# NVlabs/gbrl

Hardware: AMD Instinct MI355X
Metric: trees-fit/sec + predict rows/sec at batch=2^20, feat=128, depth=6, out=8 (higher is better)
Workload: dtype int32 fixed-point sums / f32 scores

## Files before the change

### gbrl_amd/csrc/engine_candidates.hip

```cpp
#include "engine_step_detail.h"

namespace gbrl {

namespace detail {

void spin_until_published(volatile uint32_t *flag, uint32_t seq, hipStream_t s, const char *what) {
    const double kSpinSeconds = [] { const char *e = hooks::raw(hooks::SPIN_SECONDS); const double v = e ? std::atof(e) : 0.0; return v > 0.0 ? v : 120.0; }();
    int idle = 0;
    std::chrono::steady_clock::time_point t0;
    bool timed = false;
    for (unsigned spins = 1; *flag != seq; ++spins) {
        if ((spins & 0x3fff) == 0) {
            const hipError_t q = hipStreamQuery(s);
            if (q == hipSuccess) { if (++idle > 64) throw HipError(std::string("internal: ") + what + " were not published"); }
            else if (q != hipErrorNotReady) hip_check(q, what);
            if (!timed) { t0 = std::chrono::steady_clock::now(); timed = true; }
            else if (std::chrono::duration<double>(std::chrono::steady_clock::now() - t0).count() > kSpinSeconds) {
                hip_check(hipStreamSynchronize(s), what);
                if (*flag == seq) break;
                throw HipError(std::string("timeout: ") + what + " did not arrive (stream drained, nothing published)");
            }
        }
    }
    std::atomic_thread_fence(std::memory_order_acquire);
// ... 412 lines not shown
        kern::fetch_segments(fs, s);
        cat_table_.valid = true; cat_table_.keys = d_keys; cat_table_.slot_q = d_slotq; cat_table_.cls_of_q = dc; cat_table_.log2_cap = log2_cap;
        if (cat_prof) {
            cp[4] = std::chrono::steady_clock::now();
            auto us = [](std::chrono::steady_clock::time_point a, std::chrono::steady_clock::time_point b) { return std::chrono::duration<double, std::micro>(b - a).count(); };
            fprintf(stderr, "[cat host, us] %d distinct: insertion order %.1f  items %.1f  container order %.1f  candidates + classes %.1f\n", n_distinct, us(cp[0], cp[1]), us(cp[1], cp[2]), us(cp[2], cp[3]), us(cp[3], cp[4]));
        }
        return true;
    }
    struct DictE { uint64_t h; int cls; int item; };
    std::vector<DictE> ent(n_ent);
    std::vector<int32_t> off(Fc + 1, 0);
    for (int q : cand_item) ++off[lfeat[q] + 1];
    for (int f = 0; f < Fc; ++f) off[f + 1] += off[f];
    {
        std::vector<int32_t> cur(off.begin(), off.end() - 1);
        cat_cands.reserve(cat_cands.size() + n_ent);
        for (int q : cand_item) {
            const int f = lfeat[q];
            const int cls = ++cat_classes[f];
            if (cls > 65534) throw Unsupported("more than 65534 candidate categories in one feature");
            cat_cands.emplace_back(f, cat_items_[item_of_q[q]].name, cls);
            ent[cur[f]++] = {lhash[q], cls, q};
        }
    }
    for (int f = 0; f < Fc; ++f)
        std::sort(ent.begin() + off[f], ent.begin() + off[f + 1], [](const DictE &a, const DictE &b2) { return a.h < b2.h || (a.h == b2.h && a.cls < b2.cls); });
    const size_t n1 = static_cast<size_t>(n_ent) + 1;
    const size_t o_words = 0, o_hash = o_words + n1 * kCat, o_off = o_hash + n1 * 8, o_cls = o_off + (static_cast<size_t>(Fc) + 1) * 4,
                 dict_bytes = o_cls + n1 * 4;
    char *hd = static_cast<char *>(pin_cat_dict_.ensure((dict_bytes + 3) & ~static_cast<size_t>(3)));
    for (int e = 0; e < n_ent; ++e) {
        std::memcpy(hd + o_words + static_cast<size_t>(e) * kCat, names + static_cast<size_t>(ent[e].item) * kCat, kCat);
        reinterpret_cast<uint64_t *>(hd + o_hash)[e] = ent[e].h;
        reinterpret_cast<int32_t *>(hd + o_cls)[e] = ent[e].cls;
    }
    std::memset(hd + o_words + static_cast<size_t>(n_ent) * kCat, 0, kCat);
    reinterpret_cast<uint64_t *>(hd + o_hash)[n_ent] = 0;
    reinterpret_cast<int32_t *>(hd + o_cls)[n_ent] = 0;
    std::memcpy(hd + o_off, off.data(), (static_cast<size_t>(Fc) + 1) * 4);
    char *dd = static_cast<char *>(d_sdict_.ensure((dict_bytes + 3) & ~static_cast<size_t>(3)));
    {
        void *hd_dev = nullptr;
        hip_check(hipHostGetDevicePointer(&hd_dev, hd, 0), "hipHostGetDevicePointer");
        kern::FetchSegments fs{};
        fs.n = 1; fs.dst[0] = dd; fs.src[0] = hd_dev; fs.words[0] = static_cast<uint32_t>((dict_bytes + 3) / 4);
        kern::fetch_segments(fs, s);
    }
    sdict_words_ = reinterpret_cast<const uint64_t *>(dd + o_words);
    sdict_hash_ = reinterpret_cast<const uint64_t *>(dd + o_hash);
    sdict_off_ = reinterpret_cast<const int32_t *>(dd + o_off);
    sdict_cls_ = reinterpret_cast<const int32_t *>(dd + o_cls);
    return true;
}

void Engine::verify_pending_categories() {
    bool clash = false;
    for (const auto &pq : cat_pending_) clash = clash || std::memcmp(cat_items_[pq.first].name, pq.second, kCat) != 0;
    if (!cat_pending_.empty() && hooks::on(hooks::TEST_CAT_CLASH)) clash = true;
    cat_pending_.clear();
    if (clash) cat_clash_ = true;
}

int64_t *Engine::quantile_cum_device(const std::vector<int64_t> &cum, long long n_global, int B) {
    hipStream_t s = stream_;
    const bool grown = d_cum_.capacity() < sizeof(int64_t) * static_cast<size_t>(B);
    int64_t *d_cum = static_cast<int64_t *>(d_cum_.ensure(sizeof(int64_t) * B));
    if (grown || cum_cache_n_ != n_global || cum_cache_b_ != B) {
        int64_t *h = static_cast<int64_t *>(pin_cum_.ensure(sizeof(int64_t) * B));
        std::memcpy(h, cum.data(), sizeof(int64_t) * B);
        hip_check(hipMemcpyAsync(d_cum, h, sizeof(int64_t) * B, hipMemcpyHostToDevice, s), "H2D cum");
        hip_check(hipStreamSynchronize(s), "sync cum");
        cum_cache_n_ = n_global;
        cum_cache_b_ = B;
    }
    return d_cum;
}
void Engine::numeric_thresholds(const float *dobs, int N, int F, int B, long long n_global, const uint32_t *d_kt, float *d_thr,
                                uint32_t *d_thrkeys, int pass1_chunks, uint16_t *d_codes_out, bool *codes_written) {
    if (codes_written) *codes_written = false;
    hipStream_t s = stream_;
    const gbrl_hip_metadata &md = model.meta;
    uint32_t *d_qflags = static_cast<uint32_t *>(d_qflags_.ensure(sizeof(uint32_t) * 4));
    bool fast_quantile = false;
    auto upload_cum = [&](const std::vector<int64_t> &cum) -> int64_t * { return quantile_cum_device(cum, n_global, B); };
    auto bisection_quantiles = [&](const std::vector<int64_t> &cum) {
        int64_t *d_cum = upload_cum(cum);
        uint32_t *d_prefix = static_cast<uint32_t *>(d_prefix_.ensure(sizeof(uint32_t) * F * B));
        uint32_t *d_trial = static_cast<uint32_t *>(d_trial_.ensure(sizeof(uint32_t) * F * B));
        int64_t *d_counts = static_cast<int64_t *>(d_counts_.ensure(sizeof(int64_t) * F * (B + 1)));
        kern::qsel_init(d_prefix, d_trial, F, B, s);
        for (int bit = 31; bit >= 0; --bit) {
            hip_check(hipMemsetAsync(d_counts, 0, sizeof(int64_t) * F * (B + 1), s), "memset");
            kern::bin_rows(dobs, N, F, d_trial, B, false, d_counts, nullptr, 0, 0, s);
            if (has_coll_) exchange(Red::SumI64, d_counts, static_cast<size_t>(F) * (B + 1));
            kern::qsel_update(d_prefix, d_trial, d_counts, d_cum, F, B, bit, bit - 1, s);
        }
        hip_check(hipMemcpyAsync(d_thrkeys, d_trial, sizeof(uint32_t) * F * B, hipMemcpyDeviceToDevice, s), "D2D keys");
    };
    std::vector<int64_t> cum;
    if (F > 0 && !fixed_thr_.empty()) {
        if (fixed_thr_.size() != static_cast<size_t>(F) * B) throw HipError("internal: fixed thresholds do not match this model");
        hip_check(hipMemcpyAsync(d_thr, fixed_thr_.data(), sizeof(float) * fixed_thr_.size(), hipMemcpyHostToDevice, s), "H2D thresholds");
        kern::floats_to_keys(d_thr, d_thrkeys, fixed_thr_.size(), s);
    } else if (F > 0) {
        if (md.generator_type == GBRL_HIP_GEN_UNIFORM) {
            uint32_t *d_mm = static_cast<uint32_t *>(d_minmax_.ensure(sizeof(uint32_t) * 2 * F));
            {
                kern::FillSegments fz{};
                fz.n = 2;
                fz.dst[0] = d_mm; fz.words[0] = static_cast<uint32_t>(F); fz.value[0] = 0xffffffffu;
                fz.dst[1] = d_mm + F; fz.words[1] = static_cast<uint32_t>(F); fz.value[1] = 0u;
                kern::fill_segments(fz, s);
            }
            kern::column_minmax(d_kt, N, F, d_mm, d_mm + F, s);
            if (has_coll_) {
                float *tmp = static_cast<float *>(d_trial_.ensure(sizeof(float) * 2 * F));
                kern::keys_to_floats(d_mm, tmp, 2 * static_cast<size_t>(F), s);
                kern::negate_f32(tmp, F, s);
                exchange(Red::MaxF32, tmp, 2 * static_cast<size_t>(F));
                kern::negate_f32(tmp, F, s);
                kern::floats_to_keys(tmp, d_mm, 2 * static_cast<size_t>(F), s);
            }
            kern::uniform_thresholds(d_mm, d_mm + F, F, B, d_thr, s, d_thrkeys);
        } else {
            cum = quantile_target_ranks(n_global, B);
            bool floats_done = false;
            const bool coll_fast = has_coll_ && (coll_.world_size & (coll_.world_size - 1)) == 0 && coll_.world_size <= 8;
            const bool radix_ok = !force_sample_select_ && B <= kern::radix_max_targets() && n_global < (1ll << 32);
            if (force_bisection_ || (has_coll_ && !coll_fast && !radix_ok)) {
                bisection_quantiles(cum);
            } else if (!has_coll_ && !force_sample_select_ && !force_radix_ && kern::sort_quantiles_fits(N, B)) {
                int64_t *d_cum = upload_cum(cum);
                const bool no_fuse = [] { const char *e = hooks::raw(hooks::SORT_NO_CODES); return e && e[0] == '1'; }();
                uint16_t *cdst = no_fuse ? nullptr : d_codes_out;
                kern::sort_quantiles(d_kt, N, F, d_cum, B, d_thrkeys, d_thr, s, cdst);
                if (cdst && codes_written) *codes_written = true;
                floats_done = true;
                last_quantile_fallback_ = false;
            } else if (!force_sample_select_ && B <= kern::radix_max_targets() && n_global < (1ll << 32)) {
                int64_t *d_cum = upload_cum(cum);
                void *d_rs = d_radix_state_.ensure(kern::radix_state_bytes(F, B));
                uint32_t *d_rp = static_cast<uint32_t *>(d_radix_partial_.ensure(kern::radix_partial_bytes(F)));
                uint32_t *d_rl = static_cast<uint32_t *>(d_qlists_.ensure(kern::radix_list_bytes(N, F)));
                kern::RadixComm comm{};
                if (has_coll_) {
                    comm.ctx = this;
                    comm.allreduce_sum_i64 = &Engine::radix_exchange_trampoline;
                    comm.stream_ordered = rccl_comm_ != nullptr;
                    comm.gbuf = static_cast<int64_t *>(d_counts_.ensure(sizeof(int64_t) * kern::radix_exchange_words(F)));
                    comm.partial_global = static_cast<uint32_t *>(d_radix_global_.ensure(kern::radix_global_partial_bytes(F)));
                }
                uint32_t *d_le = has_coll_ ? nullptr : static_cast<uint32_t *>(d_root_le_.ensure(sizeof(uint32_t) * (static_cast<size_t>(F) * B + F)));
                const int rc = kern::radix_select(d_kt, N, F, d_cum, B, d_rs, d_rp, d_rl, d_thrkeys, s, has_coll_ ? &comm : nullptr, pass1_chunks, d_le);
                root_le_ = d_le;
                if (rc != 0) throw HipError(rc == 2 ? "allreduce failed" : "radix select failed");
                last_quantile_fallback_ = false;
            } else {
                fast_quantile = true;
                kern::QuantilePlan plan = kern::quantile_plan(N);
                if (has_coll_) { plan.sample = 4096; plan.n_split = kern::kQuantileMaxSplit; }
                const size_t all_keys = static_cast<size_t>(N) * F;
                const uint32_t max_elems = static_cast<uint32_t>(B > 256 ? all_keys : std::min<size_t>(all_keys, std::max<size_t>(1u << 20, all_keys / 4)));
                int64_t *d_cum = upload_cum(cum);
                uint32_t *d_split = static_cast<uint32_t *>(d_splitters_.ensure(sizeof(uint32_t) * 2 * static_cast<size_t>(F) * kern::kQuantileMaxSplit));
                uint32_t *d_split_bfs = d_split + static_cast<size_t>(F) * kern::kQuantileMaxSplit;
                uint32_t *d_cc = static_cast<uint32_t *>(d_ccounts_.ensure(sizeof(uint32_t) * static_cast<size_t>(plan.n_chunks) * F * kern::kQuantileClasses));
                uint32_t *d_coff = static_cast<uint32_t *>(d_c2l_.ensure(sizeof(uint32_t) * F * kern::kQuantileClasses));
                uint32_t *d_toff = static_cast<uint32_t *>(d_tgt_list_.ensure(sizeof(uint32_t) * 2 * static_cast<size_t>(F) * B));
                uint32_t *d_tlen = d_toff + static_cast<size_t>(F) * B;
                uint32_t *d_tr = static_cast<uint32_t *>(d_tgt_rank_.ensure(sizeof(uint32_t) * F * B));
                uint32_t *d_lists = static_cast<uint32_t *>(d_qlists_.ensure(sizeof(uint32_t) * max_elems));
                hip_check(hipMemsetAsync(d_coff, 0xff, sizeof(uint32_t) * F * kern::kQuantileClasses, s), "memset");
                hip_check(hipMemsetAsync(d_qflags, 0, sizeof(uint32_t) * 4, s), "memset");
                int64_t *d_gcounts = nullptr;
                if (has_coll_) {
                    const int S = 4096, SU = S * coll_.world_size;
                    uint32_t *d_samp = static_cast<uint32_t *>(d_prefix_.ensure(sizeof(uint32_t) * static_cast<size_t>(F) * S));
                    int64_t *d_uni = static_cast<int64_t *>(d_counts_.ensure(sizeof(int64_t) * std::max<size_t>(static_cast<size_t>(F) * SU, static_cast<size_t>(F) * kern::kQuantileClasses)));
                    kern::sample_only(d_kt, N, F, S, d_samp, s);
                    hip_check(hipMemsetAsync(d_uni, 0, sizeof(int64_t) * static_cast<size_t>(F) * SU, s), "memset");
                    kern::place_sample(d_samp, F, S, coll_.rank, SU, d_uni, s);
                    exchange(Red::SumI64, d_uni, static_cast<size_t>(F) * SU);
                    kern::union_splitters(d_uni, F, SU, plan.n_split, d_split, d_split_bfs, s);
                    kern::class_count(d_kt, N, F, plan, d_split_bfs, d_cc, s);
                    d_gcounts = d_uni;
                    kern::counts_to_i64(d_cc, plan.n_chunks, static_cast<size_t>(F) * kern::kQuantileClasses, d_gcounts, s);
                    exchange(Red::SumI64, d_gcounts, static_cast<size_t>(F) * kern::kQuantileClasses);
                } else {
                    kern::sample_splitters(d_kt, N, F, plan, d_split, d_split_bfs, s);
                    hip_check(hipGetLastError(), "sample_splitters launch");
                    kern::class_count(d_kt, N, F, plan, d_split_bfs, d_cc, s);
                    hip_check(hipGetLastError(), "class_count launch");
                }
                kern::quantile_targets(d_cc, d_gcounts, d_split, d_cum, F, B, plan, d_coff, d_toff, d_tlen, d_tr, d_thrkeys, d_qflags, max_elems,
                                       d_qflags + 2, s);
                kern::quantile_extract(d_kt, N, F, plan, d_split_bfs, d_coff, d_cc, d_lists, s);
                hip_check(hipGetLastError(), "quantile_extract launch");
                if (has_coll_) {
                    uint32_t *d_pref = static_cast<uint32_t *>(d_trial_.ensure(sizeof(uint32_t) * static_cast<size_t>(F) * B));
                    int64_t *d_scnt = static_cast<int64_t *>(d_selcnt_.ensure(sizeof(int64_t) * (static_cast<size_t>(F) * B + 1)));
                    hip_check(hipMemsetAsync(d_pref, 0, sizeof(uint32_t) * static_cast<size_t>(F) * B, s), "memset");
                    for (int bit = 31; bit >= 0; --bit) {
                        kern::select_count(d_lists, d_toff, d_tlen, d_pref, bit, F * B, d_scnt, s);
                        hip_check(hipGetLastError(), "select_count launch");
                        exchange(Red::SumI64, d_scnt, static_cast<size_t>(F) * B);
                        kern::select_update(d_pref, d_scnt, d_toff, d_tr, bit, F * B, d_thrkeys, s);
                        hip_check(hipGetLastError(), "select_update launch");
                    }
                } else {
                    kern::quantile_select(d_lists, d_toff, d_tlen, d_tr, F * B, d_thrkeys, s);
                    hip_check(hipGetLastError(), "quantile_select launch");
                }
            }
            if (!floats_done) kern::keys_to_floats(d_thrkeys, d_thr, static_cast<size_t>(F) * B, s);
        }
        uint32_t qflags[4] = {0, 0, 0, 0};
        if (fast_quantile) {
            hip_check(hipMemcpyAsync(qflags, d_qflags, sizeof(qflags), hipMemcpyDeviceToHost, s), "D2H flags");
            hip_check(hipStreamSynchronize(s), "sync");
            if (has_coll_) {
                int64_t *d_flag = static_cast<int64_t *>(d_selcnt_.ensure(sizeof(int64_t) * 2));
                int64_t hv = qflags[2];
                hip_check(hipMemcpyAsync(d_flag, &hv, sizeof(hv), hipMemcpyHostToDevice, s), "H2D flag");
                exchange(Red::SumI64, d_flag, 1);
                hip_check(hipMemcpyAsync(&hv, d_flag, sizeof(hv), hipMemcpyDeviceToHost, s), "D2H flag");
                hip_check(hipStreamSynchronize(s), "sync");
                qflags[2] = hv != 0;
            }
            if (qflags[2] != 0) {
                bisection_quantiles(cum);
                kern::keys_to_floats(d_thrkeys, d_thr, static_cast<size_t>(F) * B, s);
                last_quantile_fallback_ = true;
            } else {
                last_quantile_fallback_ = false;
            }
        }
    }
}

}
```

### gbrl_amd/csrc/engine_grow_levels.hip

```cpp
#include "engine_grow_detail.h"

namespace gbrl {

using namespace detail;

void Engine::grow_levels(const GrowCtx &c, const GrowDims &dims, const StepTables &t, TreeBuilder &tb, std::vector<int64_t> &acc, double &leaf_scale) {
    hipStream_t s = stream_;
    const bool device_plan = c.oblivious && !has_coll_ && device_levels_requested() && c.MD > 0 && c.MD <= 11  &&
                             c.n_cand > 0 && !dims.l2_degenerate;
    Stager sta(pin_a_, d_stage_a_, dims.stage_bytes, s), stb(pin_b_, d_stage_b_, dims.stage_bytes, s);
    LevelWork w = level_workspace(c, dims);
    tb.reset(dims.max_nodes);
    kern::publish_pair(c.d_thr, c.pub_thr_dev, c.pub_thr_bytes, c.d_scales, c.pub_scales_dev, sizeof(kern::StepScales), s);
    if (device_plan) grow_levels_planned(c, dims, t, w, tb);
    else if (c.n_cand > 0 && !dims.l2_degenerate) grow_levels_host(c, dims, t, w, tb, sta, stb);
    finish_leaves(c, dims, w, tb, sta, acc, leaf_scale);
}

LevelWork Engine::level_workspace(const GrowCtx &c, const GrowDims &dims) {
    hipStream_t s = stream_;
    const int N = c.N, D = c.D, max_front = dims.max_front;
    LevelWork w{};
    w.rows[0] = static_cast<int32_t *>(d_rows_[0].ensure(sizeof(int32_t) * N));
    w.rows[1] = static_cast<int32_t *>(d_rows_[1].ensure(sizeof(int32_t) * N));
// ... 173 lines not shown
    L.active = std::move(active);
    const std::vector<int> &act = L.active;
    const int n_act = L.n_act = static_cast<int>(act.size());
    L.d_hist = w.hist_lvl[depth & 1];
    L.d_hist_prev = w.hist_lvl[(depth & 1) ^ 1];
    std::vector<int> &compute_ids = L.compute_ids;
    std::vector<int32_t> &slot_map = L.slot_map, sub_par(n_act, -1), sub_sib(n_act, -1);
    if (depth == 0) {
        compute_ids = act;
        for (int k = 0; k < n_act; ++k) slot_map.push_back(k);
    } else {
        std::vector<int> slot_of(nodes.size(), -1);
        for (int k = 0; k < n_act; ++k) slot_of[act[k]] = k;
        for (int k = 0; k < n_act; ++k) {
            const int id = act[k], par = nodes[id].parent;
            const int sib = nodes[par].left == id ? nodes[par].right : nodes[par].left;
            const bool sib_active = slot_of[sib] >= 0;
            const long long mine = has_coll_ ? nodes[id].n_global : nodes[id].n_local;
            const long long theirs = has_coll_ ? nodes[sib].n_global : nodes[sib].n_local;
            const bool i_am_small = sib_active && (mine < theirs || (mine == theirs && nodes[par].left == id));
            if (i_am_small) {
                compute_ids.push_back(id);
                slot_map.push_back(k);
            } else {
                sub_par[k] = nodes[par].hist_slot;
                sub_sib[k] = sib_active ? slot_of[sib] : -1;
            }
        }
    }
    for (int k = 0; k < n_act; ++k) nodes[act[k]].hist_slot = k;
    L.part_chunks = make_chunks(nodes, act, kern::kPartitionRows, false).chunks;
    if (has_coll_) L.count_chunks = L.part_chunks;
    const int direct_cap = std::min(8192, std::max(1024, 9216 / (c.D + 1)));
    L.hist_direct = !has_coll_ && !hooks::on(hooks::NO_DIRECT_HIST)  && kern::hist_direct_supported(c.FG) && !compute_ids.empty() &&
                    compute_ids.size() <= static_cast<size_t>(dims.hist_max_chunks);
    for (int id : compute_ids) L.hist_direct = L.hist_direct && nodes[id].n_local <= direct_cap;
    if (L.hist_direct) {
        L.hist.begin.assign(1, 0);
        for (size_t k = 0; k < compute_ids.size(); ++k) {
            const HNode &nd = nodes[compute_ids[k]];
            L.hist.chunks.push_back({static_cast<int32_t>(k), nd.seg_start, nd.n_local, 0});
            L.hist.begin.push_back(static_cast<int32_t>(L.hist.chunks.size()));
        }
    } else {
        L.hist = make_chunks(nodes, compute_ids, balanced_chunk_rows(nodes, compute_ids, c.chunk_rows, dims.hist_chunk_budget), false);
    }
    if (L.hist.chunks.size() > static_cast<size_t>(dims.hist_max_chunks)) throw HipError("internal: chunk table overflow");
    std::vector<int32_t> pl(n_act), ps(static_cast<size_t>(n_act) * kern::kMaxPath, -1), pb(static_cast<size_t>(n_act) * kern::kMaxPath, 0), root(n_act);
    std::vector<float> pv(static_cast<size_t>(n_act) * kern::kMaxPath, 0.f);
    std::vector<int32_t> seg_starts(n_act), n_locals(n_act);
    for (int k = 0; k < n_act; ++k) {
        const HNode &nd = nodes[act[k]];
        pl[k] = static_cast<int32_t>(nd.path.size());
        root[k] = nd.depth == 0;
        for (size_t q = 0; q < nd.path.size(); ++q) {
            ps[k * kern::kMaxPath + q] = nd.path[q].fslot;
            pv[k * kern::kMaxPath + q] = nd.path[q].value;
            pb[k * kern::kMaxPath + q] = nd.path[q].bin;
        }
        seg_starts[k] = nd.seg_start;
        n_locals[k] = nd.n_local;
    }
    sta.reset();
    L.d_chunks = sta.put(L.hist.chunks.data(), L.hist.chunks.size());
    L.d_chunk_begin = sta.put(L.hist.begin.data(), L.hist.begin.size());
    L.d_slotmap = sta.put(slot_map.data(), slot_map.size());
    L.d_sub_par = sta.put(sub_par.data(), sub_par.size());
    L.d_sub_sib = sta.put(sub_sib.data(), sub_sib.size());
    L.d_path_len = sta.put(pl.data(), pl.size());
    L.d_path_slot = sta.put(ps.data(), ps.size());
    L.d_path_val = sta.put(pv.data(), pv.size());
    L.d_path_bin = sta.put(pb.data(), pb.size());
    L.d_isroot = sta.put(root.data(), root.size());
    L.d_count_chunks = sta.put(L.count_chunks.data(), L.count_chunks.size());
    L.d_part_chunks = sta.put(L.part_chunks.data(), L.part_chunks.size());
    L.d_seg_starts = sta.put(seg_starts.data(), seg_starts.size());
    L.d_n_locals = sta.put(n_locals.data(), n_locals.size());
    sta.flush();
    L.root_mode = hooks::num(hooks::ROOT_COUNTS, 1);
    L.root_countless = depth == 0 && c.root_le != nullptr && L.root_mode != 0 && !L.hist_direct && !has_coll_ && c.n_global == c.N && c.NB == c.B + 1 &&
                       kern::hist_countless_supported(c.D, c.FG, c.N);
    L.ar_level = w.ar_prefix && sizeof(int64_t) * compute_ids.size() * dims.hist_node_elems <= dims.ar_max_bytes;
    w.ar_prefix = L.ar_level;
    L.lvl_slots = L.ar_level ? c.n_slots : dims.own_slots;
    L.lvl_lo = (has_coll_ && !L.ar_level) ? dims.coll_lo : 0;
    L.drop_derived = !has_coll_ && !hooks::on(hooks::KEEP_LAST_DERIVED)  && depth > 0 && depth == c.MD - 1;
    return L;
}

void Engine::level_histograms(const GrowCtx &c, const GrowDims &dims, const LevelWork &w, const Level &L) {
    hipStream_t s = stream_;
    const int N = c.N, F = c.F, D = c.D, B = c.B, NB = c.NB, FG = c.FG, Fp = c.Fp, n_groups = c.n_groups;
    const int n_chunks = static_cast<int>(L.hist.chunks.size()), nc = static_cast<int>(L.compute_ids.size());
    const int32_t *d_rows = w.rows[w.cur];
    int64_t *d_hist = L.d_hist;
    bool hist_written = false;
    if (n_chunks) {
        const auto ev = kernel_events("hist_build", true);
        kern::HistDirect hd;
        if (L.hist_direct) { hd.hist = d_hist; hd.slot_map = L.d_slotmap; hd.Fp = Fp; }
        hist_written = kern::hist_build(c.d_codes, N, c.d_qg, D, d_rows, L.d_chunks, n_chunks, n_groups, FG, NB, w.partials, s, ev.first, ev.second,
                                        L.hist_direct ? &hd : nullptr, !L.root_countless);
    }
    if (!hist_written) phase_begin();
    if (!has_coll_) {
        if (nc && !hist_written)
            kern::hist_reduce(w.partials, L.d_chunk_begin, L.d_slotmap, nc, n_groups, FG, NB, D, Fp, d_hist, s, n_chunks / nc, 0, L.root_countless ? c.root_le : nullptr, F, B, N);
    } else if (nc && L.ar_level) {
        bool in_place = true;
        for (int k = 0; k < nc; ++k) in_place = in_place && L.slot_map[k] == k;
        int64_t *buf = in_place ? d_hist : w.hist_coll;
        kern::hist_reduce(w.partials, L.d_chunk_begin, nullptr, nc, n_groups, FG, NB, D, Fp, buf, s, n_chunks / nc, Fp);
        exchange(Red::SumI64, buf, static_cast<size_t>(nc) * dims.hist_node_elems);
        if (!in_place) kern::hist_place(buf, d_hist, L.d_slotmap, nc, dims.hist_node_elems, s);
    } else if (nc) {
        const int coll_P = dims.coll_P, coll_Fs = dims.coll_Fs;
        if (coll_P * coll_Fs != Fp) hip_check(hipMemsetAsync(w.hist_coll, 0, sizeof(int64_t) * static_cast<size_t>(coll_P) * nc * coll_Fs * dims.feat_elems, s), "memset");
        kern::hist_reduce(w.partials, L.d_chunk_begin, nullptr, nc, n_groups, FG, NB, D, Fp, w.hist_coll, s, n_chunks / nc, coll_Fs);
        reduce_scatter_i64(w.hist_coll, w.hist_recv, static_cast<size_t>(nc) * coll_Fs * dims.feat_elems);
        kern::hist_place_slice(w.hist_recv, d_hist, L.d_slotmap, nc, coll_Fs, dims.coll_lo, Fp, dims.feat_elems, s);
    }
    if (L.root_countless && L.root_mode == 2) {
        int64_t *d_alt = w.hist_lvl[(L.depth & 1) ^ 1];
        kern::hist_build(c.d_codes, N, c.d_qg, D, d_rows, L.d_chunks, n_chunks, n_groups, FG, NB, w.partials, s, nullptr, nullptr, nullptr, true);
        kern::hist_reduce(w.partials, L.d_chunk_begin, L.d_slotmap, nc, n_groups, FG, NB, D, Fp, d_alt, s, n_chunks / nc);
        const size_t ne = dims.hist_node_elems;
        std::vector<int64_t> ha(ne), hb(ne);
        hip_check(hipMemcpyAsync(ha.data(), d_hist, ne * 8, hipMemcpyDeviceToHost, s), "D2H root histogram");
        hip_check(hipMemcpyAsync(hb.data(), d_alt, ne * 8, hipMemcpyDeviceToHost, s), "D2H root histogram");
        hip_check(hipStreamSynchronize(s), "sync");
        for (int f = 0; f < F; ++f)
            for (int cl = 0; cl < NB; ++cl)
                for (int d = 0; d <= D; ++d) {
                    const size_t i = (static_cast<size_t>(f) * NB + cl) * (D + 1) + d;
                    if (ha[i] != hb[i])
                        throw HipError("root histogram check: feature " + std::to_string(f) + " class " + std::to_string(cl) + " field " + std::to_string(d) + ": " +
                                       std::to_string(ha[i]) + " from the selection's ranks, " + std::to_string(hb[i]) + " accumulated");
                }
    }
    if (!hist_written) phase_end("hist_reduce");
}

uint32_t Engine::score_select_level(const GrowCtx &c, const GrowDims &dims, const StepTables &t, const LevelWork &w, const Level &L) {
    hipStream_t s = stream_;
    const int N = c.N, D = c.D, B = c.B, NB = c.NB, Fp = c.Fp, n_cand = c.n_cand, n_act = L.n_act, max_front = dims.max_front, depth = L.depth;
    const bool oblivious = c.oblivious, event_results = dims.event_results;
    const ResultBlock &res = w.d_res;
    phase_begin();
    if (has_coll_ && !L.ar_level && oblivious) kern::fill_f32(w.scores, static_cast<size_t>(n_act) * n_cand, -INFINITY, s);
    if (L.lvl_slots > 0)
        kern::score_candidates(L.d_hist, L.d_hist_prev, depth > 0 ? L.d_sub_par : nullptr, L.d_sub_sib, n_act, Fp, NB, D, t.slots, L.lvl_slots, c.d_thr, B, n_cand, model.meta.min_data_in_leaf, c.cosine ? 1 : 0,
                               c.d_scales, L.d_path_len, L.d_path_slot, L.d_path_val, L.d_path_bin, w.scores, w.parent, t.cand_w, t.cand_ref, L.d_isroot,
                               oblivious ? nullptr : w.am_v, w.am_i, s, L.lvl_lo, !L.drop_derived, oblivious ? nullptr : w.am_s, oblivious ? nullptr : w.am_n);
    if (oblivious)
        kern::argmax(w.scores, n_act, n_cand, t.cand_w, t.cand_ref, w.parent, L.d_isroot, oblivious, w.am_v, w.am_i, res.best_idx(), res.best_score(), s, w.am_s);
    const bool publish_in_resolve = !has_coll_ && !event_results;
    const uint32_t seq = event_results ? 0 : next_seq();
    const bool near_level = w.am_s != nullptr && publish_in_resolve;
    const kern::NearDetect near_detect{w.am_s, oblivious ? nullptr : w.am_n, dims.near_rel, w.parent, L.d_isroot, c.cosine ? 1 : 0, N};
    kern::resolve_splits(w.am_v, w.am_i, oblivious ? dims.am_parts : L.lvl_slots, res.best_idx(), res.best_score(), oblivious, n_act, t.ref_to_internal, t.cand_slot, t.slots, L.d_hist, nullptr, Fp, NB, D, w.resolved,
                         res.counts(), max_front, L.d_seg_starts, w.cursors, c.d_thrkeys, B, s, publish_in_resolve ? w.h_res_dev : nullptr, w.d_flag, seq, w.d_pub_done,
                         L.drop_derived ? L.d_hist_prev : nullptr, L.drop_derived ? L.d_sub_par : nullptr, L.drop_derived ? L.d_sub_sib : nullptr, near_level ? &near_detect : nullptr);
    if (has_coll_) {
        if (!L.ar_level) {
            const int n_win = oblivious ? 1 : n_act;
            const size_t gwords = static_cast<size_t>(dims.coll_P) * (n_win + 2 * n_act);
            kern::winner_pack(res.best_idx(), res.best_score(), res.counts(), max_front, n_win, n_act, coll_.rank, w.gather, s, dims.coll_P);
            exchange(Red::SumI64, w.gather, gwords);
            kern::winner_adopt(w.gather, dims.coll_P, n_win, n_act, oblivious, t.ref_to_internal, t.cand_slot, t.slots, L.d_seg_starts, c.d_thrkeys, B, res.best_idx(), res.best_score(),
                               res.counts(), max_front, w.resolved, w.cursors, s);
        }
        int64_t *d_right_local = res.right_local();
        if (!L.count_chunks.empty())
            kern::count_right(w.rows[w.cur], c.d_codes, c.d_kt, N, L.d_count_chunks, static_cast<int>(L.count_chunks.size()), w.resolved, d_right_local, s);
        if (event_results) kern::localize_splits(w.resolved, L.d_n_locals, d_right_local, n_act, s);
        else kern::localize_publish(w.resolved, L.d_n_locals, d_right_local, n_act, res.base, w.h_res_dev, dims.res_bytes, w.d_flag, seq, s);
    }
    if (event_results) hip_check(hipMemcpyAsync(w.h_res.base, res.base, dims.res_bytes, hipMemcpyDeviceToHost, s), "D2H level results");
    phase_end("score_select");
    return seq;
}

void Engine::replay_near_ties(const GrowCtx &c, const GrowDims &dims, const StepTables &t, const LevelWork &w, const std::vector<HNode> &nodes, const Level &L) {
    hipStream_t s = stream_;
    const int N = c.N, D = c.D, B = c.B, NB = c.NB, Fp = c.Fp, n_cand = c.n_cand, n_act = L.n_act, max_front = dims.max_front, depth = L.depth;
    const int near_max_rows = dims.near_max_rows, own_slots = dims.own_slots;
    const bool oblivious = c.oblivious, cosine = c.cosine;
    const std::vector<int> &active = L.active;
    const int64_t *near_h = w.h_res.near_flags();
    bool any = false;
    if (oblivious) {
        any = near_h[0] != 0;
        if (any && near_max_rows > 0) for (int k = 0; k < n_act; ++k) any = any && nodes[active[k]].n_local <= near_max_rows;
    } else {
        for (int k = 0; k < n_act; ++k) any = any || (near_h[k] != 0 && (near_max_rows == 0 || nodes[active[k]].n_local <= near_max_rows));
    }
    if (!any) return;
    if (hooks::on(hooks::NEARTIE_DEBUG)) {
        const float *bs = w.h_res.best_score();
        for (int k = 0; k < (oblivious ? 1 : n_act); ++k)
            if (near_h[k]) {
                const int32_t sb = static_cast<int32_t>(w.h_res.near_second()[k]);
                float sec; std::memcpy(&sec, &sb, 4);
                fprintf(stderr, "[near-tie] depth %d node %d of %d (%d rows): best gain %.9g (candidate %d), runner-up %.9g, difference %.3g\n", depth, k, n_act, nodes[active[k]].n_local,
                        bs[k], w.h_res.best_idx()[k], sec, bs[k] - sec);
            }
    }
    ++near_replays_;
    phase_begin();
    int32_t *d_cand_nr = (oblivious || N <= 8192) ? nullptr : static_cast<int32_t *>(d_near_nr_.ensure(sizeof(int32_t) * static_cast<size_t>(max_front) * std::max(1, n_cand)));
    if (!oblivious)
        kern::score_candidates(L.d_hist, L.d_hist_prev, depth > 0 ? L.d_sub_par : nullptr, L.d_sub_sib, n_act, Fp, NB, D, t.slots, own_slots, c.d_thr, B, n_cand, model.meta.min_data_in_leaf, cosine ? 1 : 0,
                               c.d_scales, L.d_path_len, L.d_path_slot, L.d_path_val, L.d_path_bin, w.scores, w.parent, t.cand_w, t.cand_ref, L.d_isroot, nullptr, w.am_i, s, 0, !L.drop_derived, nullptr, nullptr, d_cand_nr);
    kern::NearTieIO io{};
    io.rows = w.rows[w.cur]; io.seg_start = L.d_seg_starts; io.n_rows = L.d_n_locals; io.codes = c.d_codes; io.N = N; io.D = D; io.grads = c.dgrads; io.meanden = c.d_meanden;
    io.cosine = cosine ? 1 : 0; io.oblivious = oblivious ? 1 : 0; io.min_data = model.meta.min_data_in_leaf; io.slots = t.slots; io.cand_slot = t.cand_slot; io.cand_w = t.cand_w; io.cand_ref = t.cand_ref;
    io.n_cand = n_cand; io.scores = w.scores; io.cand_nr = d_cand_nr; io.parent = w.parent; io.is_root = L.d_isroot; io.best_score = w.d_res.best_score(); io.near = w.d_res.near_flags();
    io.rel = dims.near_rel; io.n_act = n_act;
    int32_t *lists = static_cast<int32_t *>(d_near_list_.ensure(sizeof(int32_t) * static_cast<size_t>(max_front) * (kern::kNearCands + 1)));
    io.list = lists; io.list_n = lists + static_cast<size_t>(max_front) * kern::kNearCands;
    io.ent = static_cast<int32_t *>(d_near_ent_.ensure(sizeof(int32_t) * std::max(static_cast<size_t>(kern::kNearCands + 1) * N, static_cast<size_t>(n_cand))));
    io.rep = static_cast<float *>(d_near_rep_.ensure(sizeof(float) * static_cast<size_t>(max_front) * (kern::kNearCands + 1)));
    io.part_v = w.am_v; io.part_i = w.am_i; io.n_parts = oblivious ? dims.am_parts : own_slots;
    io.max_node_rows = near_max_rows;
    if (const size_t mw = kern::near_tie_map_words(N, n_act)) io.maps = static_cast<uint32_t *>(d_near_maps_.ensure(sizeof(uint32_t) * mw));
    int near_largest = 0;
    for (int k = 0; k < n_act; ++k)
        if ((oblivious || near_h[k] != 0) && (near_max_rows == 0 || nodes[active[k]].n_local <= near_max_rows)) near_largest = std::max(near_largest, nodes[active[k]].n_local);
    if (kern::near_tie_fast_supported(N, D) && (reinterpret_cast<uintptr_t>(c.dgrads) & 15) == 0  && !hooks::on(hooks::NEARTIE_SERIAL) && near_largest > (cosine ? 32768 : 98304)) {
        const size_t rows17 = static_cast<size_t>(kern::kNearCands + 1) * N, blocks17 = static_cast<size_t>(n_act) * (kern::kNearCands + 1);
        io.fast = 1;
        io.pos = static_cast<int32_t *>(d_near_pos_.ensure(sizeof(int32_t) * rows17));
        io.nr = static_cast<int32_t *>(d_near_nrb_.ensure(sizeof(int32_t) * blocks17));
        io.vals = static_cast<float *>(d_near_vals_.ensure(sizeof(float) * rows17 * D));
        io.means = static_cast<float *>(d_near_means_.ensure(sizeof(float) * blocks17 * 2 * D));
        io.sums = static_cast<float *>(d_near_sums_.ensure(sizeof(float) * blocks17 * 2 * D));
        io.rowsort = static_cast<int32_t *>(d_near_rowsort_.ensure(sizeof(int32_t) * static_cast<size_t>(N)));
        io.tiles = static_cast<int32_t *>(d_near_tiles_.ensure(sizeof(int32_t) * kern::near_tie_fast_tiles(N, n_act)));
        io.seq_blocks = kern::near_tie_fast_blocks(N, D, n_act);
        io.chains_bytes = kern::near_tie_fast_chain_bytes(N, D, n_act);
        io.chains = d_near_chains_.ensure(io.chains_bytes);
    }
    kern::near_tie_replay(io, s);
    const uint32_t seq = next_seq();
    kern::resolve_splits(w.am_v, w.am_i, oblivious ? dims.am_parts : own_slots, w.d_res.best_idx(), w.d_res.best_score(), oblivious, n_act, t.ref_to_internal, t.cand_slot, t.slots, L.d_hist, nullptr, Fp, NB, D, w.resolved,
                         w.d_res.counts(), max_front, L.d_seg_starts, w.cursors, c.d_thrkeys, B, s, w.h_res_dev, w.d_flag, seq, w.d_pub_done,
                         L.drop_derived ? L.d_hist_prev : nullptr, L.drop_derived ? L.d_sub_par : nullptr, L.drop_derived ? L.d_sub_sib : nullptr, nullptr);
    if (!L.part_chunks.empty())
        kern::partition_rows(w.rows[w.cur], w.rows[w.cur ^ 1], c.d_codes, c.d_kt, N, L.d_part_chunks, static_cast<int>(L.part_chunks.size()), w.resolved, w.cursors, s);
    phase_end("near_tie_replay");
    spin_until_published(w.h_flag, seq, s, "level results after the near-tie replay");
    hip_check(hipGetLastError(), "near-tie replay kernels");
}

void Engine::finish_leaves(const GrowCtx &c, const GrowDims &dims, const LevelWork &w, TreeBuilder &tb, Stager &sta, std::vector<int64_t> &acc, double &leaf_scale) {
    hipStream_t s = stream_;
    const int D = c.D;
    std::vector<HNode> &nodes = tb.nodes;
    std::vector<int> last;
    for (int id : tb.frontier)
        if (!nodes[id].leaf) { nodes[id].leaf = true; last.push_back(id); }
    if (nodes.size() == 1) nodes[0].leaf = true;
    const ChunkTable leaves = make_chunks(nodes, last, 1024, true);
    if (!leaves.chunks.empty()) {
        sta.reset();
        Chunk *d_lc = sta.put(leaves.chunks.data(), leaves.chunks.size());
        sta.flush();
        phase_begin();
        kern::leaf_sums(c.dgrads, D, w.rows[w.cur], d_lc, static_cast<int>(leaves.chunks.size()), c.d_scales, w.leafacc, s);
        phase_end("leaves");
    }
    const size_t n_acc_words = nodes.size() * (D + 1);
    if (has_coll_) exchange(Red::SumI64, w.leafacc, n_acc_words);
    const size_t acc_bytes = sizeof(int64_t) * std::max<size_t>(1, n_acc_words);
    char *h_acc_raw = static_cast<char *>(pin_acc_.ensure(acc_bytes + 64));
    int64_t *h_acc = reinterpret_cast<int64_t *>(h_acc_raw);
    if (dims.event_results) {
        hip_check(hipMemcpyAsync(h_acc, w.leafacc, sizeof(int64_t) * n_acc_words, hipMemcpyDeviceToHost, s), "D2H leaf acc");
        hip_check(hipStreamSynchronize(s), "sync");
    } else {
        void *h_acc_dev = nullptr;
        hip_check(hipHostGetDevicePointer(&h_acc_dev, h_acc_raw, 0), "hipHostGetDevicePointer");
        volatile uint32_t *h_aflag = reinterpret_cast<volatile uint32_t *>(h_acc_raw + acc_bytes);
        const uint32_t seq = next_seq();
        *h_aflag = 0;
        kern::publish_block(w.leafacc, h_acc_dev, sizeof(int64_t) * n_acc_words, reinterpret_cast<uint32_t *>(static_cast<char *>(h_acc_dev) + acc_bytes), seq, s,
                            true);
        spin_until_published(h_aflag, seq, s, "leaf sums");
        leafacc_clean_ptr_ = w.leafacc;
    }
    acc.assign(h_acc, h_acc + n_acc_words);
    if (!std::isfinite(c.h_scales->hmax_build) || !std::isfinite(c.h_scales->hmax_raw)) throw InvalidArgument("non-finite gradients");
    leaf_scale = c.h_scales->leaf_scale;
}

}
```

### gbrl_amd/csrc/hooks.h

```cpp
#pragma once
#include <cstdlib>

namespace gbrl {
namespace hooks {

#define GBRL_HIP_HOOKS(X) \
    X(BIN_PLAIN) \
    X(CAT_CHECK) \
    X(CAT_PROF) \
    X(DEVICE_LEVELS) \
    X(EVENT_RESULTS) \
    X(FORCE_BISECTION) \
    X(FORCE_COLLECTIVE) \
    X(HIST_ALLREDUCE_MAX_KB) \
    X(HIST_GENERIC) \
    X(HIST_PIPE) \
    X(HOST_CATEGORICAL) \
    X(KEEP_LAST_DERIVED) \
    X(NEARTIE_DEBUG) \
    X(NEARTIE_MAX_ROWS) \
    X(NEARTIE_REL) \
    X(NEARTIE_SERIAL) \
    X(NO_DIRECT_HIST) \
    X(NO_IOTA_CACHE) \
    X(NO_NEARTIE_REPLAY) \
    X(NO_SMALL_GROW) \
    X(NO_SMALL_PREP) \
    X(NO_SMALL_STATS) \
    X(PREDICT_CHAIN) \
    X(PREDICT_GENERIC) \
    X(PREDICT_GRD_STREAM_MIN_ROWS) \
    X(PREDICT_GRD_STREAM_WAVES) \
    X(PREDICT_NB) \
    X(PREDICT_NOSPLIT) \
    X(PREDICT_NO_GRD_STREAM) \
    X(PREDICT_NO_PC) \
    X(PREDICT_NO_PERSIST) \
    X(PREDICT_NO_REG) \
    X(PREDICT_NO_RESIDENT) \
    X(PREDICT_OBL1) \
    X(PREDICT_REG_GROUPED) \
    X(PREDICT_REG_MIN_ROWS) \
    X(PREDICT_REG_ONLY) \
    X(PREDICT_REG_WAVES) \
    X(PREDICT_RG) \
    X(PREDICT_TT) \
    X(QUANTILE_RADIX) \
    X(QUANTILE_SAMPLE) \
    X(RADIX_PLAIN_LOADS) \
    X(ROOT_COUNTS) \
    X(SHAP_HOST) \
    X(SMALL_GROW_BLOCKS) \
    X(SMALL_GROW_PROF) \
    X(SMALL_PREP_PROF) \
    X(SORT_NO_CODES) \
    X(SPIN_SECONDS) \
    X(TEST_CAT_CLASH) \
    X(TEST_SMALL_GROW_FAIL) \
    X(TRANSPOSE_COUNT) \
    X(TRANSPOSE_PLAIN)

enum Id : int {
#define X(n) n,
    GBRL_HIP_HOOKS(X)
#undef X
    kCount
};

void begin_call();
const char *raw(Id id);
const char *name(Id id);
inline bool on(Id id) { const char *e = raw(id); return e && e[0] == '1'; }
inline int num(Id id, int dflt) { const char *e = raw(id); return e ? std::atoi(e) : dflt; }

}
}
```

### gbrl_amd/csrc/kernels.h

```cpp
#pragma once

#include <hip/hip_runtime.h>

#include <cstdint>

namespace gbrl {
namespace kern {

struct PerDeviceOnce {
    uint64_t done = 0;
    bool first() {
        int d = 0;
        if (hipGetDevice(&d) != hipSuccess || d < 0 || d >= 64) return true;
        if ((done >> d) & 1ull) return false;
        done |= 1ull << d;
        return true;
    }
};


struct Chunk {
    int32_t slot;
    int32_t start;
    int32_t len;
    int32_t pad;
};

struct FeatureSlot {
    int32_t is_cat;
    int32_t n_cand;
    int32_t cand_base;
    int32_t pad;
};

struct NodeSplit {
    int32_t do_split;
    int32_t fslot;
    int32_t bin;
    int32_t is_cat;
    int32_t seg_start;
    int32_t n_left;
    uint32_t thr_key;
    int32_t pad1;
};

struct StepScales {
    double inv_scale;
    double leaf_scale;
    float scale;
    float hmax_build;
    float hmax_raw;
    int32_t sbits, lbits, pad;
};

constexpr int kMaxPath = 32;
constexpr int kPartitionRows = 4096;

void column_sums(const float *g, int n, int D, const float *center , double *block_partials,
                 int n_blocks, double *out , hipStream_t s);
int column_sums_blocks(int n, int D);
void stats_mean(const double *stat , long long n, int D, float *meanden , hipStream_t s);
void stats_finish(const double *stat_raw , const double *stat_centred ,
                  long long n, int D, int chunk_rows, float *meanden, StepScales *sc, hipStream_t s);
bool small_stats(const float *g, int n, int D, bool centred, int chunk_rows, double *stat , float *meanden , StepScales *sc, int32_t *qg,
                 hipStream_t s);
void quantize_grads(const float *g, size_t n_el, int D, const float *mean, const float *denom, const StepScales *sc,
                    int32_t *qg, hipStream_t s);

void column_minmax(const uint32_t *kt , int n, int F, uint32_t *mn, uint32_t *mx, hipStream_t s);
void uniform_thresholds(const uint32_t *min_keys, const uint32_t *max_keys, int F, int B, float *thr, hipStream_t s,
                        uint32_t *thr_keys = nullptr );
void bin_rows(const float *obs, int n, int F, const uint32_t *trial_keys, int B, bool strict, int64_t *counts,
              uint16_t *codes, int code_stride, int code_off, hipStream_t s);
void qsel_init(uint32_t *prefix, uint32_t *trial, int F, int B, hipStream_t s);
void qsel_update(uint32_t *prefix, uint32_t *trial, const int64_t *counts, const int64_t *cum_ranks, int F, int B,
                 int bit, int next_bit, hipStream_t s);
void sub_arrays(const float *a, const float *b, float *out, size_t n, hipStream_t s);
void gather_rows(const float *src, const int32_t *perm, float *dst, int n, int width, hipStream_t s);
void f64_to_f32(const double *in, float *out, int n, hipStream_t s);
void stats_pack(const double *st, int D, int P, int rank, double *msg, hipStream_t s, double extra = 0.0);
void stats_unpack(const double *msg, int D, int P, double *st, hipStream_t s);
void negate_f32(float *p, int n, hipStream_t s);
void f32_to_f64(const float *in, double *out, int n, hipStream_t s);
void keys_to_floats(uint32_t *keys , float *out, size_t n, hipStream_t s);
void floats_to_keys(const float *in, uint32_t *keys, size_t n, hipStream_t s);
void publish_block(void *d_src, void *h_dst_mapped, size_t bytes, uint32_t *flag_mapped, uint32_t seq, hipStream_t s, bool zero_src = false );
void publish_pair(const void *d_a, void *h_a_mapped, size_t a_bytes, const void *d_b, void *h_b_mapped, size_t b_bytes, hipStream_t s);
struct FetchSegments { void *dst[8]; const void *src[8]; uint32_t words[8]; int n; };
void fetch_segments(const FetchSegments &fs, hipStream_t s);
constexpr int kStageSegments = 32;
struct StageSegments { void *dst[kStageSegments]; uint32_t src_off[kStageSegments]; uint32_t bytes[kStageSegments]; int n; };
void stage_copy(const StageSegments &ss, const void *stage_mapped, hipStream_t s);
struct FillSegments { void *dst[4]; uint32_t words[4]; uint32_t value[4]; int n; };
void fill_segments(const FillSegments &fs, hipStream_t s);
void iota_rows(int32_t *rows, int n, hipStream_t s);

struct QuantilePlan { int sample, n_split, n_chunks, chunk; };
constexpr int kQuantileClasses = 8192;
constexpr int kQuantileMaxSplit = 4095;
QuantilePlan quantile_plan(int n);
void transpose_keys(const float *obs, int n, int F, uint32_t *kt , hipStream_t s);
void sample_splitters(const uint32_t *kt, int n, int F, const QuantilePlan &p, uint32_t *splitters ,
                      uint32_t *splitters_bfs , hipStream_t s);
void class_count(const uint32_t *kt, int n, int F, const QuantilePlan &p, const uint32_t *splitters_bfs,
                 uint32_t *partial , hipStream_t s);
void quantile_targets(const uint32_t *partial, const int64_t *global_counts, const uint32_t *splitters, const int64_t *cum, int F, int B,
                      const QuantilePlan &p, uint32_t *class_off , uint32_t *tgt_off, uint32_t *tgt_len,
                      uint32_t *tgt_rank, uint32_t *thr_keys, uint32_t *alloc , uint32_t max_elems,
                      uint32_t *overflow , hipStream_t s);
void sample_only(const uint32_t *kt, int n, int F, int S, uint32_t *sample_out , hipStream_t s);
void place_sample(const uint32_t *samp, int F, int S, int rank, int SU, int64_t *uni , hipStream_t s);
void union_splitters(const int64_t *uni, int F, int SU, int n_split, uint32_t *splitters, uint32_t *splitters_bfs, hipStream_t s);
void counts_to_i64(const uint32_t *partial, int n_chunks, size_t fc, int64_t *out, hipStream_t s);
void select_count(const uint32_t *lists, const uint32_t *tgt_off, const uint32_t *tgt_len, const uint32_t *prefix, int bit, int n_targets,
                  int64_t *counts, hipStream_t s);
void select_update(uint32_t *prefix, const int64_t *counts, const uint32_t *tgt_off, const uint32_t *tgt_rank, int bit, int n_targets,
                   uint32_t *thr_keys, hipStream_t s);
void quantile_extract(const uint32_t *kt, int n, int F, const QuantilePlan &p, const uint32_t *splitters_bfs, const uint32_t *class_off,
                      const uint32_t *partial, uint32_t *out, hipStream_t s);
void quantile_select(const uint32_t *lists, const uint32_t *tgt_off, const uint32_t *tgt_len, const uint32_t *tgt_rank, int n_targets,
                     uint32_t *thr_keys, hipStream_t s);
int sort_quantiles_max_rows();
bool sort_quantiles_fits(int n, int B);
void sort_quantiles(const uint32_t *kt, int n, int F, const int64_t *cum, int B, uint32_t *thr_keys, float *thr_floats , hipStream_t s, uint16_t *codes = nullptr );
size_t radix_state_bytes(int F, int B);
size_t radix_partial_bytes(int F);
int radix_max_targets();
size_t radix_list_bytes(int n, int F);
struct RadixComm {
    void *ctx;
    int (*allreduce_sum_i64)(void *ctx, int64_t *dev_buf, size_t count);
    bool stream_ordered;
    int64_t *gbuf;
    uint32_t *partial_global;
};
size_t radix_exchange_words(int F);
size_t radix_global_partial_bytes(int F);
int radix_select(const uint32_t *kt, int n, int F, const int64_t *cum, int B, void *state, uint32_t *partial, uint32_t *lists,
                 uint32_t *thr_keys, hipStream_t s, const RadixComm *comm ,
                 int pass1_chunks = 0 ,
                 uint32_t *le_out = nullptr );
int transpose_keys_count(const float *obs, int n, int F, uint32_t *kt, uint32_t *partial, hipStream_t s);
void bin_cols(const uint32_t *kt, int n, int F, const uint32_t *thr_keys, int B, uint16_t *codes, hipStream_t s);
void scatter_cat_codes_grouped(const uint16_t *cat_codes, int n, int Fc, int F, uint16_t *codes, hipStream_t s);
constexpr int kCodeGroup = 16;

size_t hist_lds_bytes(int NB, int D, int FG);
struct HistDirect {
    int64_t *hist = nullptr;
    const int32_t *slot_map = nullptr;
    int Fp = 0;
};
bool hist_direct_supported(int FG);
bool hist_build(const uint16_t *codes, int n_rows, const int32_t *qg, int D, const int32_t *rows,
                const Chunk *chunks, int n_chunks, int n_groups, int FG, int NB, int32_t *partials, hipStream_t s,
                hipEvent_t ev_start = nullptr, hipEvent_t ev_stop = nullptr ,
                const HistDirect *direct = nullptr,
                bool count_rows = true );
bool hist_countless_supported(int D, int FG, int n_rows);
void hist_reduce(const int32_t *partials, const int32_t *slot_chunk_begin , const int32_t *slot_map, int n_slots,
                 int n_groups, int FG, int NB, int D, int Fp, int64_t *hist, hipStream_t s,
                 int chunks_per_slot = 1 ,
                 int scatter_fs = 0 ,
                 const uint32_t *root_le = nullptr ,
                 int root_F = 0, int root_B = 0, long long root_n = 0);
void hist_place_slice(const int64_t *recv, int64_t *hist, const int32_t *slot_map, int n, int fs, int lo, int Fp, size_t feat_elems, hipStream_t s);
void fill_f32(float *p, size_t n, float v, hipStream_t s);
void winner_pack(const int32_t *best_idx, const float *best_score, const int64_t *counts4, int max_front, int n_win, int n_act, int rank,
                 int64_t *gather , hipStream_t s, int P);
void winner_adopt(const int64_t *gather, int P, int n_win, int n_act, bool oblivious, const int32_t *ref_to_internal, const int32_t *cand_slot,
                  const FeatureSlot *slots, const int32_t *seg_start, const uint32_t *thr_keys, int B, int32_t *best_idx, float *best_score,
                  int64_t *counts4, int max_front, NodeSplit *out, int32_t *cursors, hipStream_t s);

void score_candidates(int64_t *hist, const int64_t *hist_prev, const int32_t *sub_par, const int32_t *sub_sib, int n_nodes, int Fp, int NB, int D, const FeatureSlot *slots, int n_slots,
                      const float *thr , int B, int n_cand, int min_data, int cosine, const StepScales *sc,
                      const int32_t *path_len, const int32_t *path_slot, const float *path_val, const int32_t *path_bin,
                      float *scores , float *parent ,
                      const float *cand_w, const int32_t *cand_ref, const int32_t *is_root,
                      float *part_v ,
                      int32_t *part_i, hipStream_t s, int slot0 = 0 ,
                      bool keep_derived = true ,
                      float *part_s = nullptr ,
                      int32_t *part_n = nullptr ,
                      int32_t *cand_nr = nullptr );
int argmax_parts(int n_cand);
void argmax(const float *scores, int n_nodes, int n_cand, const float *cand_weight, const int32_t *cand_ref, const float *parent,
            const int32_t *is_root, bool oblivious, float *part_v, int32_t *part_i, int32_t *best_idx, float *best_score,
            hipStream_t s, float *part_s = nullptr );

struct NearDetect { const float *part_s; const int32_t *part_n ; float rel; const float *parent; const int32_t *is_root; int cosine; long long rows;  };

void resolve_splits(const float *part_v, const int32_t *part_i, int n_parts ,
                    int32_t *best_idx, float *best_score, bool oblivious, int n_nodes, const int32_t *ref_to_internal, const int32_t *cand_slot,
                    const FeatureSlot *slots, const int64_t *hist_local, const int64_t *hist_global , int Fp, int NB, int D,
                    NodeSplit *out, int64_t *counts4 , int max_front,
                    const int32_t *seg_start ,
                    int32_t *cursors, const uint32_t *thr_keys , int B, hipStream_t s,
                    void *pub = nullptr ,
                    uint32_t *pub_flag = nullptr , uint32_t pub_seq = 0,
                    unsigned *pub_done = nullptr ,
                    const int64_t *hist_prev = nullptr, const int32_t *sub_par = nullptr ,
                    const int32_t *sub_sib = nullptr, const NearDetect *near = nullptr);

constexpr int kNearCands = 16;
constexpr int kNearMaxRows = 65536;
constexpr int kNearMaxD = 1024;
struct NearTieIO {
    const int32_t *rows;
    const int32_t *seg_start;
    const int32_t *n_rows;
    const uint16_t *codes;
    int N, D;
    const float *grads;
    const float *meanden;
    int cosine, oblivious, min_data;
    const FeatureSlot *slots;
    const int32_t *cand_slot;
    const float *cand_w;
    const int32_t *cand_ref;
    int n_cand;
    const float *scores;
    const int32_t *cand_nr;
    const float *parent;
    const int32_t *is_root;
    const float *best_score;
    const int64_t *near;
    float rel;
    int n_act;
    int32_t *list;
    int32_t *list_n;
    int32_t *ent;
    float *rep;
    float *part_v;
    int32_t *part_i;
    int n_parts;
    int lvl_ready;
    int fast;
    int32_t *pos;
    int32_t *nr;
    int32_t *rowsort;
    int32_t *tiles;
    float *vals;
    float *means;
    float *sums;
    void *chains;
    size_t chains_bytes;
    uint32_t seq_blocks;
    uint32_t *maps;
    int max_node_rows;
};
size_t near_tie_map_words(int N, int n_act);
bool near_tie_fast_supported(int N, int D);
uint32_t near_tie_fast_blocks(int N, int D, int n_act);
size_t near_tie_fast_chain_bytes(int N, int D, int n_act);
size_t near_tie_fast_tiles(int N, int n_act);
bool near_tie_supported(int N, int D);
void near_tie_replay(const NearTieIO &io, hipStream_t s);
bool near_tie_selftest(const float *grads, const uint8_t *in_node, const uint8_t *goes_right, int n_rows, int D, const float *meanden, bool cosine, int min_data, float *out);

struct SeqChain { const float *x; uint32_t len; uint32_t blk0; float start; };
size_t seq_sums_scratch_bytes(uint32_t n_blocks);
void seq_sums(const SeqChain *d_chains, int n_chains, uint32_t n_blocks, void *d_scratch, float *d_out, uint32_t *d_n_slow , hipStream_t s);
bool seq_sums_selftest(const float *x, const uint32_t *lens, const float *starts , int n_chains, float *out, uint32_t *n_slow_out );

void localize_splits(NodeSplit *splits, const int32_t *n_local, const int64_t *right_local, int n_nodes, hipStream_t s);
void localize_publish(NodeSplit *splits, const int32_t *n_local, const int64_t *right_local, int n_nodes, void *d_src, void *h_dst_mapped, size_t bytes,
                      uint32_t *flag_mapped, uint32_t seq, hipStream_t s);
void hist_place(const int64_t *src, int64_t *dst, const int32_t *slot_map, int n, size_t node_elems, hipStream_t s);
void count_right(const int32_t *rows, const uint16_t *codes, const uint32_t *kt , int n_rows, const Chunk *chunks, int n_chunks, const NodeSplit *splits,
                 int64_t *n_right , hipStream_t s);

struct ObliviousPlan {
    int32_t *node_seg, *node_n;
    int mf;
    Chunk *chunks; int cap_h;
    int32_t *chunk_begin;
    int32_t *slot_map, *sub_par, *sub_sib;
    int32_t *path_len, *path_slot, *path_bin, *is_root;
    float *path_val;
    Chunk *part_chunks; int cap_p;
    int32_t *seg_starts;
    int32_t *state;
    int32_t *cond_slot, *cond_bin;
    float *cond_val;
};
void plan_oblivious_level(int level, int n_rows, int chunk_rows, int budget, const NodeSplit *resolved_prev, const float *best_score_prev,
                          const float *thr, int B, const ObliviousPlan &pl, hipStream_t s);

void partition_rows(const int32_t *rows_in, int32_t *rows_out, const uint16_t *codes, const uint32_t *kt , int n_rows,
                    const Chunk *chunks, int n_chunks, const NodeSplit *splits, int32_t *cursors ,
                    hipStream_t s);

bool small_prep(const float *obs, int N, int F, int B, bool uniform, const int64_t *cum, float *thr, uint32_t *thr_keys, uint16_t *codes,
                uint16_t *codes_fm , const float *grads, int D, bool centred, int chunk_rows, double *stat, float *meanden, StepScales *sc, int32_t *qg,
                bool want_stats, bool *stats_done, hipStream_t s);

struct SmallGrowIO {
    const uint16_t *codes; const int32_t *qg; const float *grads; const StepScales *scales;
    const uint16_t *codes_fm = nullptr;
    int n_fm = 0;
    int n_thr_slots = 0;
    const FeatureSlot *slots; const float *thr; const float *cand_w; const int32_t *cand_ref;
    int N, D, B, n_slots, NB, MD, min_data;
    bool cosine, oblivious;
    int G;
    void *bests;
    unsigned *sync;
    char *res;
    char *res_dev;
    int64_t *acc;
    uint32_t *status;
    uint32_t seq;
    uint32_t *prof = nullptr;
    StepScales *scales_out = nullptr;
    void *near_scratch = nullptr;
    const float *meanden = nullptr;
    bool resume = false;
    bool replay = false;
    float near_rel = 0.0f;
};
bool small_grow_supported(int N, int D, int NB, int MD, int n_slots, int n_cand);
int small_grow_blocks(int n_slots);
size_t small_grow_bests_bytes(int MD, int G, bool oblivious);
size_t small_grow_res_stride(int MD);
size_t small_grow_near_bytes(int G, int N, int MD);
bool small_grow(const SmallGrowIO &io, hipStream_t s);

void leaf_sums(const float *grads, int D, const int32_t *rows, const Chunk *chunks, int n_chunks, const StepScales *sc,
               int64_t *acc , hipStream_t s);

struct PredictModel {
    const int32_t *tree_indices, *depths, *feature_indices, *cat_ids;
    const float *feature_values, *values, *bias;
    const uint8_t *is_numerics, *inequality_directions;
    int n_trees, n_leaves, max_depth, D, oblivious;
    int n_opts;
    const int32_t *opt_start, *opt_stop;
    const float *opt_lr;
    const int32_t *cond_pack;
    const int32_t *grd_nodes;
    const int32_t *grd_node_off;
    int grd_ok, grd_max_nodes, grd_max_leaves;
    int obl_ok, coef_ok;
    uint64_t coef_cover;
    float coef[64];
    float *partial;
    size_t partial_floats;
    int tree_chunk;
    int tree_splits;
    int par_th;
    int32_t *slots;
    size_t slot_ints;
    const float *values_sw;
    const int32_t *cond_ra;
    int obl2_maxd;
// ... 54 lines not shown
```

### gbrl_amd/csrc/kernels.hip

```cpp
#include "kernels.h"
#include "hooks.h"
#include "kernels_common.h"
#include "score_common.h"
#include "small_prep.h"

#include <hip/hip_ext.h>

#include <algorithm>
#include <cmath>
#include <stdexcept>
#include <cstdlib>

namespace gbrl {
namespace kern {

namespace {

__global__ void k_column_sums(const float *__restrict__ g, size_t n_el, int D, const float *__restrict__ center,
                              double *__restrict__ partials ) {
    extern __shared__ double sh[];
    const int bs = blockDim.x;
    const int col = threadIdx.x % D;
    const float c = center ? center[col] : 0.0f;
    double acc = 0.0;
// ... 810 lines not shown
                const int i = i0 + u * step;
                if (i < tot) { const int64_t v = a[u] - b[u]; sh64[i] = v; if (keep_derived) src[i] = v; }
            }
        }
    } else {
        const int tot = NBe * W, step = static_cast<int>(blockDim.x);
        for (int i0 = threadIdx.x; i0 < tot; i0 += kScoreLoads * step) {
            int64_t a[kScoreLoads];
#pragma unroll
            for (int u = 0; u < kScoreLoads; ++u) { const int i = i0 + u * step; a[u] = i < tot ? src[i] : 0; }
#pragma unroll
            for (int u = 0; u < kScoreLoads; ++u) { const int i = i0 + u * step; if (i < tot) sh64[i] = a[u]; }
        }
    }
    if (threadIdx.x < kWave) {
        const int p = threadIdx.x;
        const bool hit = p < kMaxPath && p < q_len && q_slot == fs;
        const unsigned long long m = __ballot(hit);
        if (hit) {
            const int pos = __popcll(m & ((1ull << p) - 1));
            s_pval[pos] = q_val;
            s_pbin[pos] = q_bin;
        }
        if (p == 0) s_np = __popcll(m);
    }
    __syncthreads();
    int64_t *total = sh64 + static_cast<size_t>(NB) * W;
    double *total_f = reinterpret_cast<double *>(total + W);
    constexpr int WCH = 9;
    __shared__ long long wsum[4][WCH];
    const int lane = threadIdx.x & (kWave - 1), wave = threadIdx.x / kWave;
    for (int w0 = 0; w0 < W; w0 += WCH) {
        long long run_base[WCH];
#pragma unroll
        for (int j = 0; j < WCH; ++j) run_base[j] = 0;
        const int n_tiles = (NBe + 255) / 256 - ((NBe % 256) != 0 && (NBe % 256) <= 4 && NBe > 256 ? 1 : 0);
        for (int tile = 0; tile < n_tiles; ++tile) {
            const int c = NBe - 1 - (tile * 256 + static_cast<int>(threadIdx.x));
            long long v[WCH];
#pragma unroll
            for (int j = 0; j < WCH; ++j) v[j] = (c >= 0 && w0 + j < W) ? sh64[c * W + w0 + j] : 0;
            static_assert(WCH == 9, "wave_scan9");
            wave_scan9(v);
            if (lane == kWave - 1) {
#pragma unroll
                for (int j = 0; j < WCH; ++j) wsum[wave][j] = v[j];
            }
            __syncthreads();
            {
                long long below[WCH], all[WCH];
#pragma unroll
                for (int j = 0; j < WCH; ++j) { below[j] = 0; all[j] = 0; }
#pragma unroll 1
                for (int i = 0; i < 4; ++i) {
#pragma unroll
                    for (int j = 0; j < WCH; ++j) { const long long x = wsum[i][j]; if (i < wave) below[j] += x; all[j] += x; }
                }
#pragma unroll
                for (int j = 0; j < WCH; ++j) {
                    if (c >= 0 && !sl.is_cat && w0 + j < W) sh64[c * W + w0 + j] = v[j] + run_base[j] + below[j];
                    run_base[j] += all[j];
                }
            }
            __syncthreads();
        }
        const int rem = NBe - n_tiles * 256;
        if (static_cast<int>(threadIdx.x) < WCH && w0 + static_cast<int>(threadIdx.x) < W) {
            const int j = threadIdx.x;
            long long run = 0;
#pragma unroll
            for (int jj = 0; jj < WCH; ++jj) if (jj == j) run = run_base[jj];
            for (int c = rem - 1; c >= 0; --c) {
                run += sh64[c * W + w0 + j];
                if (!sl.is_cat) sh64[c * W + w0 + j] = run;
            }
            total[w0 + j] = run;
            total_f[w0 + j] = static_cast<double>(run);
        }
    }
    __syncthreads();
    const int64_t n_tot = total[D];
    float par_score = 0.0f;
    if (blockIdx.x == 0 || part_v) {
        const double x = side_term(total, D, n_tot, inv_scale);
        par_score = static_cast<float>(cosine ? sqrt(x) : x);
    }
    if (blockIdx.x == 0 && threadIdx.x == 0) parent[node] = par_score;
    const float par_sub = (part_v && is_root[node]) ? 0.0f : par_score;
    Best mine{-INFINITY, 0x7fffffff};
    float second = -INFINITY;
    int mine_nr = -1;
    const int np = s_np;
    for (int k = threadIdx.x; k < sl.n_cand; k += blockDim.x) {
        const int64_t *R = sh64 + (k + 1) * W;
        const int64_t n_r = R[D], n_l = n_tot - n_r;
        bool reject = (n_l < min_data) || (n_r < min_data);
        if (np > 0) {
            const float tk = sl.is_cat ? 0.0f : thr[static_cast<size_t>(fs) * B + k];
            for (int p = 0; p < np; ++p) {
                if (sl.is_cat) reject |= (s_pbin[p] == k + 1);
                else reject |= (s_pval[p] == tk);
            }
        }
        float out;
        if (reject) {
            out = -INFINITY;
        } else {
            out = candidate_score([&](int d) { return static_cast<double>(R[d]); }, total_f, D, n_l, n_r, cosine, inv_scale);
        }
        if (part_v) {
            const int j = sl.cand_base + k;
            const float gain = fmaf(out, cand_w[j], -par_sub);
            const Best cb{gain, cand_ref[j]};
            const int cls = part_n ? near_class(n_r, n_tot) : 0;
            second = second_merge(mine.v, mine_nr, second, gain, cls, -INFINITY);
            if (better_takes_second(mine, cb)) { mine = cb; mine_nr = cls; }
        } else {
            scores[static_cast<size_t>(node) * n_cand + sl.cand_base + k] = out;
            if (cand_nr) cand_nr[static_cast<size_t>(node) * n_cand + sl.cand_base + k] = near_class(n_r, n_tot);
        }
    }
    if (part_v) {
        for (int o = kWave / 2; o > 0; o >>= 1) {
            const Best other{__shfl_xor(mine.v, o, kWave), __shfl_xor(mine.i, o, kWave)};
            if (part_s) {
                const int onr = __shfl_xor(mine_nr, o, kWave);
                second = second_merge(mine.v, mine_nr, second, other.v, onr, __shfl_xor(second, o, kWave));
                if (better_takes_second(mine, other)) mine_nr = onr;
            }
            mine = better(mine, other);
        }
        __shared__ float bv[4], b2[4];
        __shared__ int bi[4], bn[4];
        if (lane == 0) { bv[wave] = mine.v; bi[wave] = mine.i; b2[wave] = second; bn[wave] = mine_nr; }
        __syncthreads();
        if (threadIdx.x == 0) {
            Best b{bv[0], bi[0]};
            float s2 = b2[0];
            int nr = bn[0];
            for (int q = 1; q < 4; ++q) {
                const Best o{bv[q], bi[q]};
                s2 = second_merge(b.v, nr, s2, o.v, bn[q], b2[q]);
                if (better_takes_second(b, o)) { b = o; nr = bn[q]; }
            }
            part_v[static_cast<size_t>(node) * gridDim.x + blockIdx.x] = b.v;
            part_i[static_cast<size_t>(node) * gridDim.x + blockIdx.x] = b.i;
            if (part_s) part_s[static_cast<size_t>(node) * gridDim.x + blockIdx.x] = s2;
            if (part_n) part_n[static_cast<size_t>(node) * gridDim.x + blockIdx.x] = nr;
        }
    }
}

constexpr int kArgmaxThreads = 256;
__global__ __launch_bounds__(kArgmaxThreads) void k_argmax_stage1(const float *__restrict__ scores, int n_nodes, int n_cand,
                                                                  const float *__restrict__ w, const int32_t *__restrict__ ref,
                                                                  const float *__restrict__ parent, const int32_t *__restrict__ is_root,
                                                                  int oblivious, float *__restrict__ part_v, int32_t *__restrict__ part_i,
                                                                  float *__restrict__ part_s ) {
    const int j = blockIdx.x * kArgmaxThreads + threadIdx.x;
    const int node = blockIdx.y;
    Best mine{-INFINITY, 0x7fffffff};
    if (j < n_cand) {
        float sc;
        if (oblivious) {
            sc = 0.0f;
            int nd = 0;
            for (; nd + 8 <= n_nodes; nd += 8) {
                float v[8];
#pragma unroll
                for (int u = 0; u < 8; ++u) v[u] = scores[static_cast<size_t>(nd + u) * n_cand + j];
#pragma unroll
                for (int u = 0; u < 8; ++u) sc += v[u];
            }
            for (; nd < n_nodes; ++nd) sc += scores[static_cast<size_t>(nd) * n_cand + j];
            sc = sc * w[j];
        } else {
            const float par = is_root[node] ? 0.0f : parent[node];
            sc = fmaf(scores[static_cast<size_t>(node) * n_cand + j], w[j], -par);
        }
        mine = better(mine, Best{sc, ref[j]});
    }
    __shared__ float sv[kArgmaxThreads], s2[kArgmaxThreads];
    __shared__ int si[kArgmaxThreads];
    sv[threadIdx.x] = mine.v;
    si[threadIdx.x] = mine.i;
    s2[threadIdx.x] = -INFINITY;
    __syncthreads();
    for (int o = kArgmaxThreads / 2; o > 0; o >>= 1) {
        if (threadIdx.x < o) {
            Best a2{sv[threadIdx.x], si[threadIdx.x]}, b2{sv[threadIdx.x + o], si[threadIdx.x + o]};
            s2[threadIdx.x] = second_distinct(a2.v, s2[threadIdx.x], b2.v, s2[threadIdx.x + o]);
            a2 = better(a2, b2);
            sv[threadIdx.x] = a2.v;
            si[threadIdx.x] = a2.i;
        }
        __syncthreads();
    }
    if (threadIdx.x == 0) {
        part_v[static_cast<size_t>(node) * gridDim.x + blockIdx.x] = sv[0];
        part_i[static_cast<size_t>(node) * gridDim.x + blockIdx.x] = si[0];
        if (part_s) part_s[static_cast<size_t>(node) * gridDim.x + blockIdx.x] = s2[0];
    }
}
__global__ __launch_bounds__(64) void k_resolve_splits(const float *__restrict__ part_v, const int32_t *__restrict__ part_i, int n_parts,
                                                       int32_t *__restrict__ best_idx, float *__restrict__ best_score, int oblivious,
                                                       const int32_t *__restrict__ ref_to_internal, const int32_t *__restrict__ cand_slot,
                                                       const FeatureSlot *__restrict__ slots, const int64_t *__restrict__ hist_local,
                                                       const int64_t *__restrict__ hist_global, int Fp, int NB, int D,
                                                       NodeSplit *__restrict__ out, int64_t *__restrict__ counts4, int max_front,
                                                       const int32_t *__restrict__ seg_start , int32_t *__restrict__ cursors,
                                                       const uint32_t *__restrict__ thr_keys, int B, char *pub, uint32_t *pub_flag,
                                                       uint32_t pub_seq, unsigned *pub_done, const int64_t *__restrict__ hist_prev,
                                                       const int32_t *__restrict__ sub_par, const int32_t *__restrict__ sub_sib,
                                                       const float *__restrict__ part_s, const int32_t *__restrict__ part_n , float near_rel, const float *__restrict__ parent,
                                                       const int32_t *__restrict__ is_root, int cosine_score, long long near_rows) {
    const int node = blockIdx.x;
    int32_t *pub_idx = reinterpret_cast<int32_t *>(pub);
    float *pub_score = reinterpret_cast<float *>(pub + 4 * static_cast<size_t>(max_front));
    int64_t *pub_counts = reinterpret_cast<int64_t *>(pub + 8 * static_cast<size_t>(max_front));
    const int src_node = oblivious ? 0 : node;
    Best mine{-INFINITY, 0x7fffffff};
    float second = -INFINITY;
    int mine_nr = 0;
    for (int q = threadIdx.x; q < n_parts; q += kWave) {
        const Best other{part_v[static_cast<size_t>(src_node) * n_parts + q], part_i[static_cast<size_t>(src_node) * n_parts + q]};
        if (part_s) {
            const int onr = part_n ? part_n[static_cast<size_t>(src_node) * n_parts + q] : 0;
            second = second_merge(mine.v, mine_nr, second, other.v, onr, part_s[static_cast<size_t>(src_node) * n_parts + q]);
            if (better_takes_second(mine, other)) mine_nr = onr;
        }
        mine = better(mine, other);
    }
    for (int o = kWave / 2; o > 0; o >>= 1) {
        const Best other{__shfl_xor(mine.v, o, kWave), __shfl_xor(mine.i, o, kWave)};
        if (part_s) {
            const int onr = __shfl_xor(mine_nr, o, kWave);
            second = second_merge(mine.v, mine_nr, second, other.v, onr, __shfl_xor(second, o, kWave));
            if (better_takes_second(mine, other)) mine_nr = onr;
        }
        mine = better(mine, other);
    }
    const int best = mine.i == 0x7fffffff ? 0 : mine.i;
    const float best_v = mine.v;
    if (threadIdx.x == 0 && node == src_node && !hist_global) {
        counts4[3 * static_cast<size_t>(max_front) + node] = __float_as_int(second);
        if (pub) pub_counts[3 * static_cast<size_t>(max_front) + node] = __float_as_int(second);
    }
    if (threadIdx.x == 0 && node == src_node) {
        best_idx[node] = best; best_score[node] = best_v;
        if (pub) { pub_idx[node] = best; pub_score[node] = best_v; }
    }
    const int j = ref_to_internal[best];
    const int fs = cand_slot[j];
    const FeatureSlot sl = slots[fs];
    const int bin = sl.is_cat ? (j - sl.cand_base + 1) : (j - sl.cand_base);
    const int W = D + 1;
    const int NBe = min(NB, sl.n_cand + 1);
    int n_left = 0;
    for (int pass = 0; pass < (hist_global ? 2 : 1); ++pass) {
        const int64_t *src = (pass ? hist_global : hist_local) + (static_cast<size_t>(node) * Fp + fs) * NB * W;
        const int par = (sub_par && pass == 0) ? sub_par[node] : -1;
        const int64_t *sub = nullptr;
        if (par >= 0) {
            const int sib = sub_sib[node];
            src = hist_prev + (static_cast<size_t>(par) * Fp + fs) * NB * W;
            sub = sib >= 0 ? hist_local + (static_cast<size_t>(sib) * Fp + fs) * NB * W : nullptr;
        }
        long long tot = 0, right = 0;
        for (int c0 = threadIdx.x; c0 < NBe; c0 += 8 * kWave) {
            long long n[8];
#pragma unroll
            for (int u = 0; u < 8; ++u) { const int c = c0 + u * kWave; n[u] = c < NBe ? src[c * W + D] : 0; }
            if (sub) {
#pragma unroll
                for (int u = 0; u < 8; ++u) { const int c = c0 + u * kWave; n[u] -= c < NBe ? sub[c * W + D] : 0; }
            }
#pragma unroll
            for (int u = 0; u < 8; ++u) {
                const int c = c0 + u * kWave;
                tot += n[u];
                if (c < NBe && (sl.is_cat ? (c == bin) : (c > bin))) right += n[u];
            }
        }
        for (int o = kWave / 2; o > 0; o >>= 1) { tot += __shfl_xor(tot, o, kWave); right += __shfl_xor(right, o, kWave); }
        if (threadIdx.x == 0) {
            counts4[(2 * pass + 0) * static_cast<size_t>(max_front) + node] = tot;
            counts4[(2 * pass + 1) * static_cast<size_t>(max_front) + node] = right;
            if (pub) {
                pub_counts[(2 * pass + 0) * static_cast<size_t>(max_front) + node] = tot;
                pub_counts[(2 * pass + 1) * static_cast<size_t>(max_front) + node] = right;
            }
            if (pass == 0) n_left = static_cast<int>(tot - right);
            if (pass == 0 && !hist_global) {
                long long near = 0;
                if (part_s && best_v != -INFINITY && node == src_node) {
                    float mag;
                    if (oblivious) mag = fabsf(best_v);
                    else { const float par = is_root[node] ? 0.0f : parent[node]; mag = fmaxf(fabsf(best_v + par), fabsf(par)); }
                    const float win = near_window_rel(near_rel, oblivious ? near_rows : tot) * mag;
                    if (second != -INFINITY && best_v - second <= win) near = 1;
                    if (!oblivious && !is_root[node] && fabsf(best_v) <= win && !(cosine_score == 0 && (right == 0 || right == tot))) near = 1;
                }
                counts4[2 * static_cast<size_t>(max_front) + node] = near;
                if (pub) pub_counts[2 * static_cast<size_t>(max_front) + node] = near;
            }
        }
    }
    if (threadIdx.x == 0) {
        NodeSplit q{};
        q.fslot = fs; q.bin = bin; q.is_cat = sl.is_cat;
        q.thr_key = (!sl.is_cat && thr_keys) ? thr_keys[static_cast<size_t>(fs) * B + bin] : 0u;
        if (seg_start) {
            const float bs = best_v;
            q.do_split = oblivious ? (bs != -INFINITY) : (bs >= 0.0f);
            q.seg_start = seg_start[node];
            q.n_left = n_left;
            cursors[2 * node] = 0;
            cursors[2 * node + 1] = 0;
        }
        out[node] = q;
        if (pub) {
            __threadfence_system();
            if (atomicAdd(pub_done, 1u) == gridDim.x - 1) {
                *pub_done = 0;
                __hip_atomic_store(pub_flag, pub_seq, __ATOMIC_RELEASE, __HIP_MEMORY_SCOPE_SYSTEM);
            }
        }
    }
}

constexpr int kPartThreads = 1024;
constexpr int kPartRows = 4096;
__global__ __launch_bounds__(kPartThreads) void k_partition(const int32_t *__restrict__ rows_in, int32_t *__restrict__ rows_out,
                                                            const uint16_t *__restrict__ codes, const uint32_t *__restrict__ kt, int n_rows,
                                                            const Chunk *__restrict__ chunks, const NodeSplit *__restrict__ splits,
                                                            int32_t *__restrict__ cursors) {
    const Chunk ck = chunks[blockIdx.x];
    if (ck.len <= 0) return;
    const NodeSplit sp = splits[ck.slot];
    if (!sp.do_split) return;
    const int lane = threadIdx.x & (kWave - 1);
    constexpr int U = kPartRows / kPartThreads;
    int row[U];
    bool right[U];
#pragma unroll
    for (int u = 0; u < U; ++u) {
        const int p = u * kPartThreads + threadIdx.x;
        row[u] = p < ck.len ? rows_in[ck.start + p] : -1;
    }
    if (!sp.is_cat && kt) {
        const uint32_t *kcol = kt + static_cast<size_t>(sp.fslot) * n_rows;
#pragma unroll
        for (int u = 0; u < U; ++u) right[u] = row[u] >= 0 && kcol[row[u]] > sp.thr_key;
    } else {
        const uint16_t *cbase = codes + (static_cast<size_t>(sp.fslot >> 4) * n_rows) * kCodeGroup + (sp.fslot & (kCodeGroup - 1));
#pragma unroll
        for (int u = 0; u < U; ++u) {
            const int code = row[u] >= 0 ? cbase[static_cast<size_t>(row[u]) * kCodeGroup] : 0;
            right[u] = sp.is_cat ? (code == sp.bin) : (code > sp.bin);
        }
    }
    const unsigned long long below = (lane == 0) ? 0ull : (~0ull >> (kWave - lane));
    constexpr int W = kPartThreads / kWave;
    __shared__ int cnt[W * U][2];
    __shared__ int base[2];
    const int wave = threadIdx.x / kWave;
    unsigned long long mr[U], ml[U];
#pragma unroll
    for (int u = 0; u < U; ++u) {
        const bool active = row[u] >= 0;
        mr[u] = __ballot(active && right[u]);
        ml[u] = __ballot(active && !right[u]);
        if (lane == 0) { cnt[wave * U + u][1] = __popcll(mr[u]); cnt[wave * U + u][0] = __popcll(ml[u]); }
    }
    __syncthreads();
    if (threadIdx.x < 2) {
        const int side = threadIdx.x;
        int run = 0;
        for (int q = 0; q < W * U; ++q) { const int c = cnt[q][side]; cnt[q][side] = run; run += c; }
        base[side] = run ? atomicAdd(&cursors[ck.slot * 2 + side], run) : 0;
    }
    __syncthreads();
#pragma unroll
    for (int u = 0; u < U; ++u) {
        if (row[u] < 0) continue;
        const int off = cnt[wave * U + u][right[u] ? 1 : 0];
        const int dst = right[u] ? (sp.seg_start + sp.n_left + base[1] + off + __popcll(mr[u] & below))
                                 : (sp.seg_start + base[0] + off + __popcll(ml[u] & below));
        rows_out[dst] = row[u];
    }
}

__global__ __launch_bounds__(kPartThreads) void k_count_right(const int32_t *__restrict__ rows, const uint16_t *__restrict__ codes,
                                                              const uint32_t *__restrict__ kt, int n_rows, const Chunk *__restrict__ chunks,
                                                              const NodeSplit *__restrict__ splits, int64_t *__restrict__ n_right) {
    const Chunk ck = chunks[blockIdx.x];
    const NodeSplit sp = splits[ck.slot];
    const uint16_t *cbase = codes + (static_cast<size_t>(sp.fslot >> 4) * n_rows) * kCodeGroup + (sp.fslot & (kCodeGroup - 1));
    int c = 0;
    if (!sp.is_cat && kt) {
        const uint32_t *kcol = kt + static_cast<size_t>(sp.fslot) * n_rows;
        for (int p = threadIdx.x; p < ck.len; p += kPartThreads) c += kcol[rows[ck.start + p]] > sp.thr_key ? 1 : 0;
    } else {
        for (int p = threadIdx.x; p < ck.len; p += kPartThreads) {
            const int code = cbase[static_cast<size_t>(rows[ck.start + p]) * kCodeGroup];
            c += (sp.is_cat ? (code == sp.bin) : (code > sp.bin)) ? 1 : 0;
        }
    }
    for (int o = kWave / 2; o > 0; o >>= 1) c += __shfl_xor(c, o, kWave);
    __shared__ int wsum[kPartThreads / kWave];
    if ((threadIdx.x & (kWave - 1)) == 0) wsum[threadIdx.x / kWave] = c;
    __syncthreads();
    if (threadIdx.x == 0) {
        long long tot = 0;
        for (int w = 0; w < kPartThreads / kWave; ++w) tot += wsum[w];
        if (tot) atomicAdd(reinterpret_cast<unsigned long long *>(&n_right[ck.slot]), static_cast<unsigned long long>(tot));
    }
}

__global__ __launch_bounds__(256) void k_leaf_sums(const float *__restrict__ grads, int D, const int32_t *__restrict__ rows,
                                                   const Chunk *__restrict__ chunks, const StepScales *__restrict__ scp,
                                                   int64_t *__restrict__ acc) {
    extern __shared__ unsigned long long shl[];
    const double scale = scp->leaf_scale;
    for (int i = threadIdx.x; i <= D; i += blockDim.x) shl[i] = 0ull;
    __syncthreads();
    const Chunk ck = chunks[blockIdx.x];
    const int per = blockDim.x / D > 0 ? blockDim.x / D : 1;
    const int d = threadIdx.x % D, sub = threadIdx.x / D;
    long long s = 0;
    if (sub < per) {
        int p = sub;
        for (; p + 7 * per < ck.len; p += 8 * per) {
            int r[8];
            float g[8];
#pragma unroll
            for (int u = 0; u < 8; ++u) r[u] = rows[ck.start + p + u * per];
#pragma unroll
            for (int u = 0; u < 8; ++u) g[u] = grads[static_cast<size_t>(r[u]) * D + d];
#pragma unroll
            for (int u = 0; u < 8; ++u) s += __double2ll_rn(static_cast<double>(g[u]) * scale);
        }
        for (; p < ck.len; p += per) {
            const int row = rows[ck.start + p];
            s += __double2ll_rn(static_cast<double>(grads[static_cast<size_t>(row) * D + d]) * scale);
        }
        atomicAdd(&shl[d], static_cast<unsigned long long>(s));
    }
    __syncthreads();
    for (int i = threadIdx.x; i < D; i += blockDim.x)
        atomicAdd(reinterpret_cast<unsigned long long *>(&acc[static_cast<size_t>(ck.slot) * (D + 1) + i]), shl[i]);
    if (threadIdx.x == 0)
        atomicAdd(reinterpret_cast<unsigned long long *>(&acc[static_cast<size_t>(ck.slot) * (D + 1) + D]),
                  static_cast<unsigned long long>(ck.len));
}

}


int column_sums_blocks(int n, int D) { return grid_for(static_cast<size_t>(n) * D, 256 * 8, 1024); }

void column_sums(const float *g, int n, int D, const float *center, double *block_partials, int n_blocks, double *out,
                 hipStream_t s) {
    const int bs = D <= 256 ? (256 / D) * D : D;
    hipLaunchKernelGGL(k_column_sums, dim3(n_blocks), dim3(bs), 2 * bs * sizeof(double), s, g, static_cast<size_t>(n) * D, D,
                       center, block_partials);
    hipLaunchKernelGGL(k_column_sums_final, dim3(2 * D), dim3(256), 0, s, block_partials, n_blocks, D, out);
}

bool small_stats(const float *g, int n, int D, bool centred, int chunk_rows, double *stat, float *meanden, StepScales *sc, int32_t *qg, hipStream_t s) {
    const int n_blocks = column_sums_blocks(n, D);
    const int bs = D <= 256 ? (256 / D) * D : D;
    if (D > 16 || n_blocks * bs > kSmallStatsVirtual || n_blocks > 32 || n < 2) return false;
    const size_t lds = sizeof(double) * (2 * static_cast<size_t>(n_blocks) * bs + static_cast<size_t>(n_blocks) * 2 * D);
    if (lds > 156 * 1024) return false;
    static PerDeviceOnce attr;
    static uint64_t unsupported = 0;
    int dev = 0;
    (void)hipGetDevice(&dev);
    const uint64_t bit = (dev >= 0 && dev < 64) ? (1ull << dev) : 0;
// ... 197 lines not shown
                    int n_chunks, int n_groups, int NB, int32_t *partials, size_t lds, hipStream_t s, hipEvent_t ev_start, hipEvent_t ev_stop) {
        if (r == R) {
            constexpr int U = R <= 8 ? 4 : 2;
            static PerDeviceOnce attr_set;
            if (attr_set.first()) {
                (void)hipFuncSetAttribute(reinterpret_cast<const void *>(k_hist_build_quad<R, U>), hipFuncAttributeMaxDynamicSharedMemorySize,
                                          160 * 1024);
            }
            const int grid = 8 * n_groups * ((n_chunks + 7) / 8);
            hipExtLaunchKernelGGL((k_hist_build_quad<R, U>), dim3(grid), dim3(kHistThreads), lds, s, ev_start, ev_stop, 0, codes, n_rows, qg,
                                  D, rows, chunks, n_chunks, n_groups, NB, partials);
            return true;
        }
        return QuadDispatch<R - 1>::run(r, codes, n_rows, qg, D, rows, chunks, n_chunks, n_groups, NB, partials, lds, s, ev_start, ev_stop);
    }
};
template <>
struct QuadDispatch<0> {
    static bool run(int, const uint16_t *, int, const int32_t *, int, const int32_t *, const Chunk *, int, int, int, int32_t *, size_t,
                    hipStream_t, hipEvent_t, hipEvent_t) { return false; }
};

static bool launch_hist_wide(int P, int H, const uint16_t *codes, int n_rows, const int32_t *qg, int D, const int32_t *rows,
                             const Chunk *chunks, int n_chunks, int n_groups, int NB, int32_t *partials, size_t lds, hipStream_t s,
                             hipEvent_t ev_start, hipEvent_t ev_stop) {
    if (H < 1 || H > 16) return false;
    if (P == 2) return WideDispatch<2, 16>::run(H, codes, n_rows, qg, D, rows, chunks, n_chunks, n_groups, NB, partials, lds, s, ev_start, ev_stop);
    return false;
}

bool hist_direct_supported(int FG) { return FG != 8 && FG != 4; }
bool hist_countless_supported(int D, int FG, int n_rows) {
    const bool generic_only = [] { const char *e = hooks::raw(hooks::HIST_GENERIC); return e && e[0] == '1'; }();
    const bool pipe = [] { const char *e = hooks::raw(hooks::HIST_PIPE); return !(e && e[0] == '0'); }();
    return !generic_only && pipe && FG == 16 && D >= 1 && D <= 16 && n_rows <= (1 << 26);
}
bool hist_build(const uint16_t *codes, int n_rows, const int32_t *qg, int D, const int32_t *rows, const Chunk *chunks,
                int n_chunks, int n_groups, int FG, int NB, int32_t *partials, hipStream_t s, hipEvent_t ev_start, hipEvent_t ev_stop,
                const HistDirect *direct, bool count_rows) {
    const HistDirect dir = direct ? *direct : HistDirect{};
    int shift = 0;
    while ((1 << shift) < FG) ++shift;
    const size_t lds = hist_lds_bytes(NB, D, FG);
    const bool generic_only = [] { const char *e = hooks::raw(hooks::HIST_GENERIC); return e && e[0] == '1'; }();
    if (generic_only || n_rows > (1 << 26)) {
        launch_hist<0, 4>(codes, n_rows, qg, D, rows, chunks, n_chunks, n_groups, FG, shift, NB, partials, lds, s, ev_start, ev_stop, dir);
        return dir.hist != nullptr;
    }
#ifndef GBRL_HIST_U
#define GBRL_HIST_U 8
#endif
#define GBRL_HIST_CASE(DD) case DD: launch_hist<DD, GBRL_HIST_U>(codes, n_rows, qg, D, rows, chunks, n_chunks, n_groups, FG, shift, NB, partials, lds, s, ev_start, ev_stop, dir, count_rows); return dir.hist != nullptr;
    if (FG == 16) {
        switch (D) {
            GBRL_HIST_CASE(1) GBRL_HIST_CASE(2) GBRL_HIST_CASE(3) GBRL_HIST_CASE(4) GBRL_HIST_CASE(5) GBRL_HIST_CASE(6)
            GBRL_HIST_CASE(7) GBRL_HIST_CASE(8) GBRL_HIST_CASE(9) GBRL_HIST_CASE(10) GBRL_HIST_CASE(11) GBRL_HIST_CASE(12)
            GBRL_HIST_CASE(13) GBRL_HIST_CASE(14) GBRL_HIST_CASE(15) GBRL_HIST_CASE(16)
            default: break;
        }
    }
#undef GBRL_HIST_CASE
    if (FG == 8 && D + 1 <= 32) {
        if (launch_hist_wide(2, (D + 2) / 2, codes, n_rows, qg, D, rows, chunks, n_chunks, n_groups, NB, partials, lds, s, ev_start, ev_stop)) return false;
    }
    if (FG == 4 && D + 1 <= 64) {
        if (QuadDispatch<16>::run((D + 4) / 4, codes, n_rows, qg, D, rows, chunks, n_chunks, n_groups, NB, partials, lds, s, ev_start, ev_stop)) return false;
    }
    launch_hist<0, 4>(codes, n_rows, qg, D, rows, chunks, n_chunks, n_groups, FG, shift, NB, partials, lds, s, ev_start, ev_stop, dir);
    return dir.hist != nullptr;
}

void hist_reduce(const int32_t *partials, const int32_t *slot_chunk_begin, const int32_t *slot_map, int n_slots, int n_groups, int FG,
                 int NB, int D, int Fp, int64_t *hist, hipStream_t s, int chunks_per_slot, int scatter_fs, const uint32_t *root_le, int root_F,
                 int root_B, long long root_n) {
    const int n_acc = NB * (D + 1) * FG;
    dim3 grid((n_acc + 255) / 256, n_groups, n_slots);
    if (FG != 16) root_le = nullptr;
    if (chunks_per_slot >= 48)
        hipLaunchKernelGGL(k_hist_reduce<4>, grid, dim3(256, 4), 0, s, partials, slot_chunk_begin, slot_map, n_groups, FG, NB, D, Fp, hist, scatter_fs, root_le, root_F, root_B, root_n);
    else
        hipLaunchKernelGGL(k_hist_reduce<1>, grid, dim3(256, 1), 0, s, partials, slot_chunk_begin, slot_map, n_groups, FG, NB, D, Fp, hist, scatter_fs, root_le, root_F, root_B, root_n);
}
void hist_place_slice(const int64_t *recv, int64_t *hist, const int32_t *slot_map, int n, int fs, int lo, int Fp, size_t feat_elems, hipStream_t s) {
    if (n <= 0 || fs <= 0) return;
    hipLaunchKernelGGL(k_hist_place_slice, dim3(static_cast<unsigned>(std::max<size_t>(1, std::min<size_t>(8, (feat_elems + 255) / 256))), fs, n), dim3(256), 0, s, recv, hist,
                       slot_map, fs, lo, Fp, feat_elems);
}
void publish_block(void *d_src, void *h_dst_mapped, size_t bytes, uint32_t *flag_mapped, uint32_t seq, hipStream_t s, bool zero_src) {
    hipLaunchKernelGGL(k_publish_block, dim3(1), dim3(256), 0, s, static_cast<uint32_t *>(d_src), static_cast<uint32_t *>(h_dst_mapped),
                       static_cast<int>(bytes / 4), flag_mapped, seq, zero_src ? 1 : 0);
}
void publish_pair(const void *d_a, void *h_a_mapped, size_t a_bytes, const void *d_b, void *h_b_mapped, size_t b_bytes, hipStream_t s) {
    const int aw = static_cast<int>(a_bytes / 4), bw = static_cast<int>(b_bytes / 4);
    hipLaunchKernelGGL(k_publish_pair, dim3((std::max(aw, bw) + 255) / 256), dim3(256), 0, s, static_cast<const uint32_t *>(d_a),
                       static_cast<uint32_t *>(h_a_mapped), aw, static_cast<const uint32_t *>(d_b), static_cast<uint32_t *>(h_b_mapped), bw);
}
void fetch_segments(const FetchSegments &fs, hipStream_t s) {
    uint32_t mx = 0;
    for (int k = 0; k < fs.n; ++k) mx = std::max(mx, fs.words[k]);
    if (mx) hipLaunchKernelGGL(k_fetch_segments, dim3((mx + 255) / 256), dim3(256), 0, s, fs);
}
void stage_copy(const StageSegments &ss, const void *stage_mapped, hipStream_t s) {
    uint32_t mx = 0;
    for (int k = 0; k < ss.n; ++k) mx = std::max(mx, ss.bytes[k]);
    if (!mx || ss.n <= 0) return;
    const unsigned bx = std::min<unsigned>(64, (mx / 4 + 255) / 256 + 1);
    hipLaunchKernelGGL(k_stage_copy, dim3(bx, ss.n), dim3(256), 0, s, ss, static_cast<const char *>(stage_mapped));
}
void fill_segments(const FillSegments &fs, hipStream_t s) {
    uint32_t mx = 0;
    for (int k = 0; k < fs.n; ++k) mx = std::max(mx, fs.words[k]);
    if (mx) hipLaunchKernelGGL(k_fill_segments, dim3((mx + 255) / 256), dim3(256), 0, s, fs);
}
void fill_f32(float *p, size_t n, float v, hipStream_t s) {
    if (n) hipLaunchKernelGGL(k_fill_f32, dim3(static_cast<unsigned>((n + 255) / 256)), dim3(256), 0, s, p, n, v);
}
void winner_pack(const int32_t *best_idx, const float *best_score, const int64_t *counts4, int max_front, int n_win, int n_act, int rank,
                 int64_t *gather, hipStream_t s, int P) {
    hipLaunchKernelGGL(k_winner_pack, dim3((n_act + 63) / 64), dim3(64), 0, s, best_idx, best_score, counts4, max_front, n_win, n_act, rank, gather, P);
}
void winner_adopt(const int64_t *gather, int P, int n_win, int n_act, bool oblivious, const int32_t *ref_to_internal, const int32_t *cand_slot,
                  const FeatureSlot *slots, const int32_t *seg_start, const uint32_t *thr_keys, int B, int32_t *best_idx, float *best_score,
                  int64_t *counts4, int max_front, NodeSplit *out, int32_t *cursors, hipStream_t s) {
    hipLaunchKernelGGL(k_winner_adopt, dim3((n_act + 63) / 64), dim3(64), 0, s, gather, P, n_win, n_act, oblivious ? 1 : 0, ref_to_internal, cand_slot,
                       slots, seg_start, thr_keys, B, best_idx, best_score, counts4, max_front, out, cursors);
}

void score_candidates(int64_t *hist, const int64_t *hist_prev, const int32_t *sub_par, const int32_t *sub_sib, int n_nodes, int Fp, int NB,
                      int D, const FeatureSlot *slots, int n_slots,
                      const float *thr, int B, int n_cand, int min_data, int cosine, const StepScales *sc,
                      const int32_t *path_len, const int32_t *path_slot, const float *path_val, const int32_t *path_bin,
                      float *scores, float *parent, const float *cand_w, const int32_t *cand_ref, const int32_t *is_root, float *part_v,
                      int32_t *part_i, hipStream_t s, int slot0, bool keep_derived, float *part_s, int32_t *part_n, int32_t *cand_nr) {
    const size_t lds = static_cast<size_t>(NB + 2) * (D + 1) * sizeof(int64_t);
    static PerDeviceOnce attr_set;
    if (attr_set.first()) {
        (void)hipFuncSetAttribute(reinterpret_cast<const void *>(k_score), hipFuncAttributeMaxDynamicSharedMemorySize, 150 * 1024);
    }
    hipLaunchKernelGGL(k_score, dim3(n_slots, n_nodes), dim3(256), lds, s, hist, hist_prev, sub_par, sub_sib, Fp, NB, D, slots, thr, B, n_cand, min_data,
                       cosine, sc, path_len, path_slot, path_val, path_bin, scores, parent, cand_w, cand_ref, is_root, part_v, part_i, slot0,
                       keep_derived ? 1 : 0, part_s, part_n, cand_nr);
}

int argmax_parts(int n_cand) { return (n_cand + kArgmaxThreads - 1) / kArgmaxThreads; }
void argmax(const float *scores, int n_nodes, int n_cand, const float *w, const int32_t *ref, const float *parent,
            const int32_t *is_root, bool oblivious, float *part_v, int32_t *part_i, int32_t *best_idx, float *best_score,
            hipStream_t s, float *part_s) {
    const int parts = argmax_parts(n_cand);
    const int out_nodes = oblivious ? 1 : n_nodes;
    hipLaunchKernelGGL(k_argmax_stage1, dim3(parts, out_nodes), dim3(kArgmaxThreads), 0, s, scores, n_nodes, n_cand, w, ref, parent,
                       is_root, oblivious ? 1 : 0, part_v, part_i, part_s);
    (void)best_idx; (void)best_score;
}
void resolve_splits(const float *part_v, const int32_t *part_i, int n_parts, int32_t *best_idx, float *best_score, bool oblivious, int n_nodes, const int32_t *ref_to_internal, const int32_t *cand_slot,
                    const FeatureSlot *slots, const int64_t *hist_local, const int64_t *hist_global, int Fp, int NB, int D,
                    NodeSplit *out, int64_t *counts4, int max_front, const int32_t *seg_start, int32_t *cursors, const uint32_t *thr_keys,
                    int B, hipStream_t s, void *pub, uint32_t *pub_flag, uint32_t pub_seq, unsigned *pub_done, const int64_t *hist_prev,
                    const int32_t *sub_par, const int32_t *sub_sib, const NearDetect *near) {
    hipLaunchKernelGGL(k_resolve_splits, dim3(n_nodes), dim3(64), 0, s, part_v, part_i, n_parts, best_idx, best_score, oblivious ? 1 : 0,
                       ref_to_internal, cand_slot, slots, hist_local, hist_global, Fp, NB, D, out, counts4, max_front, seg_start, cursors, thr_keys, B,
                       static_cast<char *>(pub), pub_flag, pub_seq, pub_done, hist_prev, sub_par, sub_sib,
                       near ? near->part_s : nullptr, near ? near->part_n : nullptr, near ? near->rel : 0.0f, near ? near->parent : nullptr, near ? near->is_root : nullptr, near ? near->cosine : 1, near ? near->rows : 0);
}

__global__ void k_localize_splits(NodeSplit *__restrict__ splits, const int32_t *__restrict__ n_local,
                                  const int64_t *__restrict__ right_local, int n_nodes) {
    const int k = blockIdx.x * blockDim.x + threadIdx.x;
    if (k < n_nodes) splits[k].n_left = n_local[k] - static_cast<int32_t>(right_local[k]);
}
void localize_splits(NodeSplit *splits, const int32_t *n_local, const int64_t *right_local, int n_nodes, hipStream_t s) {
    hipLaunchKernelGGL(k_localize_splits, dim3((n_nodes + 63) / 64), dim3(64), 0, s, splits, n_local, right_local, n_nodes);
}
__global__ __launch_bounds__(256) void k_localize_publish(NodeSplit *__restrict__ splits, const int32_t *__restrict__ n_local, const int64_t *__restrict__ right_local,
                                                          int n_nodes, const uint32_t *__restrict__ src, uint32_t *__restrict__ dst, int words, uint32_t *flag, uint32_t seq) {
    for (int k = threadIdx.x; k < n_nodes; k += 256) splits[k].n_left = n_local[k] - static_cast<int32_t>(right_local[k]);
    for (int i = threadIdx.x; i < words; i += 256) __builtin_nontemporal_store(src[i], &dst[i]);
    __threadfence_system();
    __syncthreads();
    if (threadIdx.x == 0) __hip_atomic_store(flag, seq, __ATOMIC_RELEASE, __HIP_MEMORY_SCOPE_SYSTEM);
}
void localize_publish(NodeSplit *splits, const int32_t *n_local, const int64_t *right_local, int n_nodes, void *d_src, void *h_dst_mapped, size_t bytes,
                      uint32_t *flag_mapped, uint32_t seq, hipStream_t s) {
    hipLaunchKernelGGL(k_localize_publish, dim3(1), dim3(256), 0, s, splits, n_local, right_local, n_nodes, static_cast<const uint32_t *>(d_src),
                       static_cast<uint32_t *>(h_dst_mapped), static_cast<int>(bytes / 4), flag_mapped, seq);
}
__global__ void k_hist_place(const int64_t *__restrict__ src, int64_t *__restrict__ dst, const int32_t *__restrict__ slot_map,
                             size_t node_elems) {
    const int32_t slot = slot_map[blockIdx.y];
    for (size_t i = static_cast<size_t>(blockIdx.x) * blockDim.x + threadIdx.x; i < node_elems;
         i += static_cast<size_t>(gridDim.x) * blockDim.x)
        dst[static_cast<size_t>(slot) * node_elems + i] = src[static_cast<size_t>(blockIdx.y) * node_elems + i];
}
void hist_place(const int64_t *src, int64_t *dst, const int32_t *slot_map, int n, size_t node_elems, hipStream_t s) {
    const int bx = static_cast<int>(std::min<size_t>(256, (node_elems + 255) / 256));
    hipLaunchKernelGGL(k_hist_place, dim3(bx, n), dim3(256), 0, s, src, dst, slot_map, node_elems);
}

void count_right(const int32_t *rows, const uint16_t *codes, const uint32_t *kt, int n_rows, const Chunk *chunks, int n_chunks,
                 const NodeSplit *splits, int64_t *n_right, hipStream_t s) {
    hipLaunchKernelGGL(k_count_right, dim3(n_chunks), dim3(kPartThreads), 0, s, rows, codes, kt, n_rows, chunks, splits, n_right);
}

constexpr int kPlanThreads = 256;
constexpr int kPlanMaxNodes = 1024;
__global__ __launch_bounds__(kPlanThreads) void k_plan_oblivious(int L, int n_rows, int chunk_rows, int budget, const NodeSplit *__restrict__ prev,
                                                                 const float *__restrict__ best_prev, const float *__restrict__ thr, int B, ObliviousPlan pl) {
    __shared__ int s_seg[kPlanMaxNodes], s_cnt[kPlanMaxNodes], s_small[kPlanMaxNodes / 2 + 1], s_cb[kPlanMaxNodes / 2 + 2], s_pb[kPlanMaxNodes + 1];
    __shared__ int s_stopped, s_t, s_cslot[kMaxPath], s_cbin[kMaxPath];
    __shared__ float s_cval[kMaxPath];
    const int tid = threadIdx.x;
    const int n_act = 1 << L, n_comp = L == 0 ? 1 : n_act / 2;
    if (tid == 0) {
        int stopped = 0;
        if (L > 0) {
            stopped = pl.state[0] != 0;
            if (!stopped && best_prev[0] == -INFINITY) { stopped = 1; pl.state[0] = 1; pl.state[1] = L - 1; }
        } else {
            pl.state[0] = 0; pl.state[1] = -1;
        }
        s_stopped = stopped;
    }
#pragma unroll 1
    for (int q = tid; q < L - 1; q += kPlanThreads) { s_cslot[q] = pl.cond_slot[q]; s_cbin[q] = pl.cond_bin[q]; s_cval[q] = pl.cond_val[q]; }
    __syncthreads();
    const bool stopped = s_stopped != 0;
    if (L == 0) {
        if (tid == 0) { s_seg[0] = 0; s_cnt[0] = n_rows; }
    } else {
        const int32_t *pseg = pl.node_seg + static_cast<size_t>(L - 1) * pl.mf, *pcnt = pl.node_n + static_cast<size_t>(L - 1) * pl.mf;
    #pragma unroll 1
        for (int k = tid; k < n_act / 2; k += kPlanThreads) {
            const int nl = stopped ? 0 : prev[k].n_left, ps = stopped ? 0 : pseg[k], pc = stopped ? 0 : pcnt[k];
            s_seg[2 * k] = ps; s_cnt[2 * k] = nl;
            s_seg[2 * k + 1] = ps + nl; s_cnt[2 * k + 1] = pc - nl;
        }
        if (tid == 0 && !stopped) {
            const NodeSplit c = prev[0];
            s_cslot[L - 1] = c.fslot;
            s_cbin[L - 1] = c.bin;
            s_cval[L - 1] = c.is_cat ? INFINITY : thr[static_cast<size_t>(c.fslot) * B + c.bin];
            pl.cond_slot[L - 1] = s_cslot[L - 1]; pl.cond_bin[L - 1] = s_cbin[L - 1]; pl.cond_val[L - 1] = s_cval[L - 1];
        }
    }
    __syncthreads();
    int32_t *seg = pl.node_seg + static_cast<size_t>(L) * pl.mf, *cnt = pl.node_n + static_cast<size_t>(L) * pl.mf;
#pragma unroll 1
    for (int k = tid; k < n_act; k += kPlanThreads) { seg[k] = s_seg[k]; cnt[k] = s_cnt[k]; pl.seg_starts[k] = s_seg[k]; }
    if (L == 0) {
        if (tid == 0) { s_small[0] = 0; pl.slot_map[0] = 0; pl.sub_par[0] = -1; pl.sub_sib[0] = -1; }
    } else {
    #pragma unroll 1
        for (int p = tid; p < n_comp; p += kPlanThreads) {
            const int l = 2 * p, r = 2 * p + 1;
            const int small = s_cnt[l] <= s_cnt[r] ? l : r, big = small == l ? r : l;
            s_small[p] = small;
            pl.slot_map[p] = small;
            pl.sub_par[small] = -1; pl.sub_sib[small] = -1;
            pl.sub_par[big] = stopped ? -1 : p; pl.sub_sib[big] = stopped ? -1 : small;
        }
    }
    __syncthreads();
    auto parts_at = [&](int t) {
        int q = 0;
#pragma unroll 1
        for (int p = 0; p < n_comp; ++p) q += (s_cnt[s_small[p]] + t - 1) / t;
        return q;
    };
    {
        const int lo = min(1024, chunk_rows), hi = chunk_rows;
        const int step = max(1, (hi - lo + kPlanThreads - 1) / kPlanThreads);
        if (tid == 0) s_t = hi;
        __syncthreads();
        const int tc = min(hi, lo + tid * step);
        if (parts_at(tc) <= budget) atomicMin(&s_t, tc);
        __syncthreads();
        const int coarse = s_t;
        __syncthreads();
        if (coarse > lo) {
            const int tf = coarse - step + 1 + tid;
            if (tf >= lo && tf < coarse && parts_at(tf) <= budget) atomicMin(&s_t, tf);
        }
        __syncthreads();
    }
#pragma unroll 1
    for (int p = tid; p < n_comp; p += kPlanThreads) s_cb[p + 1] = (s_cnt[s_small[p]] + s_t - 1) / s_t;
#pragma unroll 1
    for (int k = tid; k < n_act; k += kPlanThreads) s_pb[k + 1] = (s_cnt[k] + kPartitionRows - 1) / kPartitionRows;
    __syncthreads();
    if (tid == 0) {
        int nc = 0;
        s_cb[0] = 0;
    #pragma unroll 1
        for (int p = 0; p < n_comp; ++p) { nc = min(pl.cap_h, nc + s_cb[p + 1]); s_cb[p + 1] = nc; }
        int np = 0;
        s_pb[0] = 0;
    #pragma unroll 1
        for (int k = 0; k < n_act; ++k) { np = min(pl.cap_p, np + s_pb[k + 1]); s_pb[k + 1] = np; }
    }
    __syncthreads();
    const int t = s_t;
#pragma unroll 1
    for (int p = tid; p <= n_comp; p += kPlanThreads) pl.chunk_begin[p] = s_cb[p];
#pragma unroll 1
    for (int i = tid; i < pl.cap_h; i += kPlanThreads) {
        Chunk ck{0, 0, 0, 0};
        if (i < s_cb[n_comp]) {
            int lo = 0, hi = n_comp - 1;
#pragma unroll 1
            while (lo < hi) { const int mid = (lo + hi + 1) >> 1; if (s_cb[mid] <= i) lo = mid; else hi = mid - 1; }
            const int p = lo, n = s_cnt[s_small[p]], parts = (n + t - 1) / t, each = parts ? (n + parts - 1) / parts : 0;
            const int off = (i - s_cb[p]) * each;
            if (off < n) ck = Chunk{p, s_seg[s_small[p]] + off, min(each, n - off), 0};
        }
        pl.chunks[i] = ck;
    }
// ... 44 lines not shown
```

### gbrl_amd/csrc/radix_select.hip

```cpp
#include "kernels.h"
#include "hooks.h"

#include <algorithm>
#include <cstdlib>
#include <vector>

namespace gbrl {
namespace kern {

namespace {

constexpr int kBins1 = 4096;
constexpr int kNone = 0xffff;
constexpr int kRadixThreads = 1024;
constexpr int kMaxTargets = 256;
constexpr int kChunks1 = 8;
constexpr int kCopies1 = 4;
constexpr int kChunksN = 8;
constexpr int kFiltWords = 1024, kFiltShift = 17;
constexpr int kSlotStride = 128;

__host__ __device__ constexpr int radix_bins(int pass) { return pass == 1 ? kBins1 : (pass == 4 ? 64 : 128); }
__host__ __device__ constexpr int radix_shift(int pass) { return pass == 1 ? 20 : (pass == 2 ? 13 : (pass == 3 ? 6 : 0)); }

struct RadixState {
    uint16_t *map1;
    uint16_t *child_off;
    uint64_t *child_bits;
    uint32_t *n_slots;
    uint16_t *tgt_slot;
    uint32_t *tgt_rank;
    uint32_t *tgt_prefix;
    uint32_t *list_cnt;
    uint32_t *lists;
    uint32_t list_cap;
};

template <int PASS>
__global__ __launch_bounds__(kRadixThreads) void k_radix_count(const uint32_t *__restrict__ kt, int n, int n_chunks, int B,
                                                               RadixState st, uint32_t *__restrict__ partial, bool plain_loads) {
    extern __shared__ uint32_t rl[];
    constexpr int NB = radix_bins(PASS);
    constexpr int SH = radix_shift(PASS);
    const int f = blockIdx.y;
    const int n_slots = PASS == 1 ? kCopies1 : static_cast<int>(st.n_slots[f * 4 + (PASS - 2)]);
    const int n_cnt = n_slots * NB;
    uint32_t *cnt = rl;
    uint16_t *map1 = reinterpret_cast<uint16_t *>(rl + (PASS == 1 ? kCopies1 * kBins1 : kMaxTargets * NB));
    uint64_t *cbits = reinterpret_cast<uint64_t *>(map1 + kBins1);
    uint16_t *coff = reinterpret_cast<uint16_t *>(cbits + 2 * 512);
    uint32_t *filt = reinterpret_cast<uint32_t *>(coff + 2 * 260);
    uint32_t *queue = filt + kFiltWords + (threadIdx.x >> 6) * 128;
    constexpr int PS = PASS == 3 ? 13 : 6;
    __shared__ uint32_t list_cursor;
    if (threadIdx.x == 0) list_cursor = 0;
    uint32_t *my_list = st.lists + (static_cast<size_t>(f) * n_chunks + blockIdx.x) * st.list_cap;
    for (int i = threadIdx.x; i < n_cnt; i += kRadixThreads) cnt[i] = 0;
    if (PASS >= 3) {
        for (int i = threadIdx.x; i < kFiltWords; i += kRadixThreads) filt[i] = 0;
        __syncthreads();
        if (static_cast<int>(threadIdx.x) < B) {
            const uint32_t h = ((st.tgt_prefix[static_cast<size_t>(f) * B + threadIdx.x] >> PS) * 0x9E3779B1u) >> kFiltShift;
            atomicOr(&filt[h >> 5], 1u << (h & 31));
        }
    }
    if (PASS >= 2) {
        const uint32_t *src = reinterpret_cast<const uint32_t *>(st.map1 + static_cast<size_t>(f) * kBins1);
        for (int i = threadIdx.x; i < kBins1 / 2; i += kRadixThreads) reinterpret_cast<uint32_t *>(map1)[i] = src[i];
    }
    if (PASS >= 3) {
        const int levels = PASS - 2;
        for (int i = threadIdx.x; i < levels * 258; i += kRadixThreads) coff[i] = st.child_off[static_cast<size_t>(f) * 2 * 258 + i];
        for (int i = threadIdx.x; i < levels * 512; i += kRadixThreads) cbits[i] = st.child_bits[static_cast<size_t>(f) * 2 * 512 + i];
    }
    __syncthreads();
    const uint32_t *col = kt + static_cast<size_t>(f) * n;
    const int chunk = ((n + n_chunks - 1) / n_chunks + 3) & ~3;
    const int lo = blockIdx.x * chunk, hi = min(n, lo + chunk);
    auto child = [&](int level, int slot, int digit) -> int {
        const uint64_t w0 = cbits[level * 512 + slot * 2], w1 = cbits[level * 512 + slot * 2 + 1];
        const uint64_t w = digit & 64 ? w1 : w0;
        const int bit = digit & 63;
        if (!((w >> bit) & 1)) return kNone;
        const int below = __popcll(w & ((1ull << bit) - 1)) + (digit & 64 ? __popcll(w0) : 0);
        return coff[level * 258 + slot] + below;
    };
    auto count_one = [&](uint32_t key) {
        int slot = PASS == 1 ? static_cast<int>(__lane_id() & (kCopies1 - 1)) : 0;
        if (PASS >= 2) {
            slot = map1[key >> 20];
            if (PASS >= 3 && slot != kNone) slot = child(0, slot, (key >> 13) & 127);
            if (PASS >= 4 && slot != kNone) slot = child(1, slot, (key >> 6) & 127);
        }
        const int idx = slot == kNone ? -1 : slot * NB + static_cast<int>((key >> SH) & (NB - 1));
        if (PASS == 3) {
            const unsigned long long m = __ballot(idx >= 0);
            if (m) {
                const int leader = __ffsll(static_cast<long long>(m)) - 1;
                uint32_t base = 0;
                if (static_cast<int>(__lane_id()) == leader) base = atomicAdd(&list_cursor, static_cast<uint32_t>(__popcll(m)));
                base = __builtin_amdgcn_readlane(base, leader);
                if (idx >= 0) {
                    const uint32_t pos = base + __popcll(m & ((1ull << __lane_id()) - 1));
                    if (pos < st.list_cap) my_list[pos] = key;
                }
            }
        }
        const int first = __builtin_amdgcn_readfirstlane(idx);
        const unsigned long long active = __ballot(1);
        const unsigned long long same = __ballot(idx == first);
        if (same == active) {
            if (first >= 0 && __lane_id() == static_cast<unsigned>(__ffsll(static_cast<long long>(active)) - 1))
                atomicAdd(&cnt[first], static_cast<uint32_t>(__popcll(active)));
        } else if (idx >= 0) {
            atomicAdd(&cnt[idx], 1u);
        }
    };
    constexpr int U = 16;
    int i0 = lo + threadIdx.x;
    int qlen = 0;
    if (PASS == 4) {
        const uint32_t n_list = st.list_cnt[f * n_chunks + blockIdx.x];
        if (n_list <= st.list_cap) {
            for (uint32_t i = threadIdx.x; i < n_list; i += kRadixThreads) count_one(my_list[i]);
            i0 = hi;
        }
    }
    auto strip = [&](const uint32_t (&key)[U]) __attribute__((always_inline)) {
        if (PASS >= 3) {
#pragma unroll
            for (int u = 0; u < U; ++u) {
                const uint32_t h = ((key[u] >> PS) * 0x9E3779B1u) >> kFiltShift;
                const bool hit = (filt[h >> 5] >> (h & 31)) & 1;
                const unsigned long long m = __ballot(hit);
                if (m) {
                    if (hit) queue[qlen + __popcll(m & ((1ull << __lane_id()) - 1))] = key[u];
                    qlen += __popcll(m);
                    __builtin_amdgcn_wave_barrier();
                    if (qlen >= 64) {
                        const uint32_t k0 = queue[__lane_id()];
                        const uint32_t k1 = queue[64 + __lane_id()];
                        count_one(k0);
                        qlen -= 64;
                        if (static_cast<int>(__lane_id()) < qlen) queue[__lane_id()] = k1;
                        __builtin_amdgcn_wave_barrier();
                    }
                }
            }
        } else {
#pragma unroll
            for (int u = 0; u < U; ++u) count_one(key[u]);
        }
    };
    if (i0 < hi && (n & 3) == 0 && !plain_loads) {
        const int iters = (hi - i0 + static_cast<int>(threadIdx.x)) / (kRadixThreads * U);
        const uint4 *c4 = reinterpret_cast<const uint4 *>(col + (i0 - static_cast<int>(threadIdx.x)));
        for (int it = 0; it < iters; ++it) {
            uint32_t key[U];
#pragma unroll
            for (int v = 0; v < U / 4; ++v) {
                const uint4 x = c4[(it * (U / 4) + v) * kRadixThreads + threadIdx.x];
                key[4 * v] = x.x; key[4 * v + 1] = x.y; key[4 * v + 2] = x.z; key[4 * v + 3] = x.w;
            }
            strip(key);
        }
        i0 += iters * kRadixThreads * U;
    }
    for (; i0 - static_cast<int>(__lane_id()) + 63 + (U - 1) * kRadixThreads < hi; i0 += kRadixThreads * U) {
        uint32_t key[U];
#pragma unroll
        for (int u = 0; u < U; ++u) key[u] = col[i0 + u * kRadixThreads];
        strip(key);
    }
    if (PASS >= 3 && static_cast<int>(__lane_id()) < qlen) count_one(queue[__lane_id()]);
    for (; i0 < hi; i0 += kRadixThreads) count_one(col[i0]);
    __syncthreads();
    if (PASS == 3 && threadIdx.x == 0) st.list_cnt[f * n_chunks + blockIdx.x] = list_cursor;
    uint32_t *dst = partial + (static_cast<size_t>(f) * n_chunks + blockIdx.x) * (PASS == 1 ? kBins1 : kMaxTargets * kSlotStride);
    if (PASS == 1) {
        for (int i = threadIdx.x; i < kBins1; i += kRadixThreads) {
            uint32_t v = 0;
#pragma unroll
            for (int c = 0; c < kCopies1; ++c) v += cnt[c * kBins1 + i];
            dst[i] = v;
        }
    } else {
        for (int i = threadIdx.x; i < n_cnt; i += kRadixThreads) dst[(i / NB) * kSlotStride + (i % NB)] = cnt[i];
    }
}

constexpr int kTcThreads = 1024;
constexpr int kTcWaves = kTcThreads / 64;
constexpr int kTcWaveRows = 16;
constexpr int kTcPatch = 20;
constexpr int kTcChunk = 32768;
constexpr int kTcMaxChunks = 128;
constexpr int kTcDepth = 2;

__device__ __forceinline__ uint32_t tc_float_to_key(float x) {
    uint32_t u = __float_as_uint(x);
    if ((u << 1) == 0) u = 0;
    if ((u & 0x7fffffffu) > 0x7f800000u) return 0u;
    return (u & 0x80000000u) ? ~u : (u | 0x80000000u);
}

__global__ __launch_bounds__(kTcThreads) void k_transpose_count(const float *__restrict__ obs, int n, int F, uint32_t *__restrict__ kt,
                                                                uint16_t *__restrict__ partial16, int n_chunks) {
    extern __shared__ uint32_t tc_lds[];
    constexpr int CW = kBins1 / 2;
    uint32_t *cnt = tc_lds;
    const int chunk = blockIdx.x, f0 = blockIdx.y * 16;
    const int tid = threadIdx.x, wave = tid >> 6, lane = tid & 63;
    uint32_t *patch = tc_lds + 16 * CW + wave * (16 * kTcPatch);
    {
        uint4 *c4 = reinterpret_cast<uint4 *>(cnt);
        for (int i = tid; i < 16 * CW / 4; i += kTcThreads) c4[i] = make_uint4(0, 0, 0, 0);
    }
    const int r_lo = chunk * kTcChunk, r_hi = min(n, r_lo + kTcChunk);
    const int lr = lane >> 2, q = lane & 3;
    const int sf = lane >> 2, sq = lane & 3;
    const bool fq_ok = f0 + 4 * q < F;
    const int fq = fq_ok ? f0 + 4 * q : 0;
    constexpr int kStep = kTcWaveRows * kTcWaves;
    auto load = [&](int r) -> float4 { return *reinterpret_cast<const float4 *>(obs + static_cast<size_t>(min(r, n - 1)) * F + fq); };
    int g = r_lo + wave * kTcWaveRows;
    float4 buf[kTcDepth];
#pragma unroll
    for (int d = 0; d < kTcDepth; ++d) buf[d] = load(g + d * kStep + lr);
    __syncthreads();
    uint32_t *cbase = cnt + (4 * q) * CW;
    for (; g < r_hi; g += kStep) {
        const float4 cur = buf[0];
#pragma unroll
        for (int d = 0; d + 1 < kTcDepth; ++d) buf[d] = buf[d + 1];
        buf[kTcDepth - 1] = load(g + kTcDepth * kStep + lr);
        const uint32_t k0 = tc_float_to_key(cur.x), k1 = tc_float_to_key(cur.y), k2 = tc_float_to_key(cur.z), k3 = tc_float_to_key(cur.w);
        uint32_t *t = patch + (4 * q) * kTcPatch + lr;
        t[0] = k0; t[kTcPatch] = k1; t[2 * kTcPatch] = k2; t[3 * kTcPatch] = k3;
        if (g + lr < r_hi && fq_ok) {
            atomicAdd(cbase + (k0 >> 21), 1u << ((k0 >> 16) & 16));
            atomicAdd(cbase + CW + (k1 >> 21), 1u << ((k1 >> 16) & 16));
            atomicAdd(cbase + 2 * CW + (k2 >> 21), 1u << ((k2 >> 16) & 16));
            atomicAdd(cbase + 3 * CW + (k3 >> 21), 1u << ((k3 >> 16) & 16));
        }
        __builtin_amdgcn_wave_barrier();
        const uint4 o = *reinterpret_cast<const uint4 *>(patch + sf * kTcPatch + 4 * sq);
        __builtin_amdgcn_wave_barrier();
        if (f0 + sf < F && g + 4 * sq < r_hi)
            *reinterpret_cast<uint4 *>(kt + static_cast<size_t>(f0 + sf) * n + g + 4 * sq) = o;
    }
    __syncthreads();
    for (int i = tid; i < 16 * CW / 4; i += kTcThreads) {
        const int fl = i / (CW / 4);
        if (f0 + fl < F) {
            uint4 *dst = reinterpret_cast<uint4 *>(partial16 + (static_cast<size_t>(f0 + fl) * n_chunks + chunk) * kBins1);
            dst[i % (CW / 4)] = reinterpret_cast<const uint4 *>(cnt)[i];
        }
    }
}

constexpr int kTgtThreads = 1024;

__device__ __forceinline__ uint32_t wave_scan_incl(uint32_t v) {
    const int lane = threadIdx.x & 63;
#pragma unroll
    for (int d = 1; d < 64; d <<= 1) { const uint32_t t = __shfl_up(v, d); if (lane >= d) v += t; }
    return v;
}
__device__ __forceinline__ uint32_t block_scan_incl(uint32_t v, uint32_t *scratch ) {
    const int lane = threadIdx.x & 63, w = threadIdx.x >> 6;
    v = wave_scan_incl(v);
    if (lane == 63) scratch[w] = v;
    __syncthreads();
    uint32_t base = 0;
    for (int i = 0; i < w; ++i) base += scratch[i];
    __syncthreads();
    return v + base;
}

__global__ __launch_bounds__(kTgtThreads) void k_radix_targets(int pass, const uint32_t *__restrict__ partial, int n_chunks,
                                                               const int64_t *__restrict__ cum, int B, RadixState st,
                                                               uint32_t *__restrict__ thr_keys, int p1_u16, uint32_t *__restrict__ le_out,
                                                               const int64_t *__restrict__ gbuf , int F) {
    extern __shared__ uint32_t sums[];
    __shared__ int tslot[kMaxTargets], tdig[kMaxTargets];
    __shared__ uint32_t scratch[16], total_slots;
    const int f = blockIdx.x, k = threadIdx.x, lane = threadIdx.x & 63, wave = threadIdx.x >> 6;
    const int NB = radix_bins(pass);
    const int n_slots = pass == 1 ? 1 : static_cast<int>(st.n_slots[f * 4 + (pass - 2)]);
    const size_t pstride = pass == 1 ? kBins1 : kMaxTargets * kSlotStride;
    const uint32_t *p0 = partial + static_cast<size_t>(f) * n_chunks * pstride;
    if (pass == 1) {
        uint4 v = make_uint4(0, 0, 0, 0);
        if (gbuf) {
            v = *reinterpret_cast<const uint4 *>(gbuf + static_cast<size_t>(f) * (kBins1 / 2) + 2 * k);
        } else if (p1_u16) {
            const uint16_t *q0 = reinterpret_cast<const uint16_t *>(partial) + static_cast<size_t>(f) * n_chunks * kBins1 + k * 4;
            int c = 0;
            for (; c + 8 <= n_chunks; c += 8) {
                uint2 t[8];
#pragma unroll
                for (int u = 0; u < 8; ++u) t[u] = *reinterpret_cast<const uint2 *>(q0 + static_cast<size_t>(c + u) * kBins1);
#pragma unroll
                for (int u = 0; u < 8; ++u) { v.x += t[u].x & 0xffffu; v.y += t[u].x >> 16; v.z += t[u].y & 0xffffu; v.w += t[u].y >> 16; }
            }
            for (; c < n_chunks; ++c) {
                const uint2 t = *reinterpret_cast<const uint2 *>(q0 + static_cast<size_t>(c) * kBins1);
                v.x += t.x & 0xffffu; v.y += t.x >> 16; v.z += t.y & 0xffffu; v.w += t.y >> 16;
            }
        } else
        for (int c = 0; c < n_chunks; ++c) {
            const uint4 t = *reinterpret_cast<const uint4 *>(p0 + c * pstride + k * 4);
            v.x += t.x; v.y += t.y; v.z += t.z; v.w += t.w;
        }
        v.y += v.x; v.z += v.y; v.w += v.z;
        const uint32_t base = block_scan_incl(v.w, scratch) - v.w;
        sums[k * 4 + 0] = base + v.x; sums[k * 4 + 1] = base + v.y; sums[k * 4 + 2] = base + v.z; sums[k * 4 + 3] = base + v.w;
    } else {
        for (int row = wave; row < n_slots; row += kTgtThreads / 64) {
            uint32_t a = 0, b = 0;
            if (gbuf) {
                if (2 * lane < NB) {
                    const uint2 t = *reinterpret_cast<const uint2 *>(gbuf + (static_cast<size_t>(row) * F + f) * (NB / 2) + lane);
                    a = t.x; b = t.y;
                }
            } else if (2 * lane < NB)
                for (int c = 0; c < n_chunks; ++c) {
                    const uint2 t = *reinterpret_cast<const uint2 *>(p0 + c * pstride + row * kSlotStride + 2 * lane);
                    a += t.x; b += t.y;
                }
            const uint32_t incl = wave_scan_incl(a + b);
            if (2 * lane < NB) { sums[row * NB + 2 * lane] = incl - b; sums[row * NB + 2 * lane + 1] = incl; }
        }
    }
    __syncthreads();
    int slot = 0, digit = 0;
    uint32_t rank = 0, prefix = 0;
    if (k < B) {
        if (pass == 1) {
            rank = static_cast<uint32_t>(cum[k]);
        } else {
            slot = st.tgt_slot[static_cast<size_t>(f) * B + k];
            rank = st.tgt_rank[static_cast<size_t>(f) * B + k];
            prefix = st.tgt_prefix[static_cast<size_t>(f) * B + k];
        }
        const uint32_t *hs = sums + slot * NB;
        int lo = 0, hi = NB - 1;
        while (lo < hi) { const int mid = (lo + hi) >> 1; if (hs[mid] < rank) lo = mid + 1; else hi = mid; }
        digit = lo;
        if (pass == 1 && k == 0 && le_out) le_out[static_cast<size_t>(gridDim.x) * B + f] = sums[7];
        const uint32_t le_here = static_cast<uint32_t>(static_cast<uint64_t>(cum[k]) - rank + hs[lo]);
        rank -= lo ? hs[lo - 1] : 0u;
        prefix |= static_cast<uint32_t>(digit) << radix_shift(pass);
        if (pass == 4 && le_out) le_out[static_cast<size_t>(f) * B + k] = prefix < 0x007fffffu ? le_out[static_cast<size_t>(gridDim.x) * B + f] : le_here;
    }
    if (pass == 4) {
        if (k < B) thr_keys[static_cast<size_t>(f) * B + k] = prefix;
        return;
    }
    if (k < kMaxTargets) { tslot[k] = k < B ? slot : -1; tdig[k] = digit; }
    __syncthreads();
    const bool opens = (k < B) && (k == 0 || tslot[k - 1] != slot || tdig[k - 1] != digit);
    const bool new_parent = (k < B) && (k == 0 || tslot[k - 1] != slot);
    const uint32_t incl = block_scan_incl(opens ? 1u : 0u, scratch);
    const int my_slot = static_cast<int>(incl) - 1;
    if (k == B - 1) total_slots = incl;
    if (k < B) {
        st.tgt_slot[static_cast<size_t>(f) * B + k] = static_cast<uint16_t>(my_slot);
        st.tgt_rank[static_cast<size_t>(f) * B + k] = rank;
        st.tgt_prefix[static_cast<size_t>(f) * B + k] = prefix;
    }
    if (pass == 1) {
        uint16_t *m = st.map1 + static_cast<size_t>(f) * kBins1;
        for (int i = threadIdx.x; i < kBins1; i += kTgtThreads) m[i] = kNone;
        __syncthreads();
        if (opens) m[digit] = static_cast<uint16_t>(my_slot);
    } else {
        uint16_t *off = st.child_off + (static_cast<size_t>(f) * 2 + (pass - 2)) * 258;
        unsigned long long *bits = reinterpret_cast<unsigned long long *>(st.child_bits) + (static_cast<size_t>(f) * 2 + (pass - 2)) * 512;
        for (int i = threadIdx.x; i < 2 * n_slots; i += kTgtThreads) bits[i] = 0ull;
        __syncthreads();
        if (opens) atomicOr(&bits[slot * 2 + (digit >> 6)], 1ull << (digit & 63));
        if (new_parent) off[slot] = static_cast<uint16_t>(my_slot);
    }
    __syncthreads();
    if (k == 0) st.n_slots[f * 4 + (pass - 1)] = total_slots;
}

__global__ __launch_bounds__(256) void k_radix_globalize(int pass, const uint32_t *__restrict__ partial, int n_chunks, int F,
                                                         RadixState st, int64_t *__restrict__ gbuf, int p1_u16) {
    const int NB = radix_bins(pass), NBh = NB / 2;
    const int rows = pass == 1 ? 1 : kMaxTargets;
    const size_t pstride = pass == 1 ? kBins1 : kMaxTargets * kSlotStride;
    const size_t total = static_cast<size_t>(rows) * F * NBh;
    for (size_t i = static_cast<size_t>(blockIdx.x) * blockDim.x + threadIdx.x; i < total; i += static_cast<size_t>(gridDim.x) * blockDim.x) {
        const int pair = static_cast<int>(i % NBh);
        const int f = static_cast<int>((i / NBh) % F);
        const int slot = static_cast<int>(i / (static_cast<size_t>(NBh) * F));
        uint32_t a = 0, b = 0;
        const int live = pass == 1 ? 1 : static_cast<int>(st.n_slots[f * 4 + (pass - 2)]);
        if (p1_u16 && pass == 1) {
            const uint16_t *p = reinterpret_cast<const uint16_t *>(partial) + static_cast<size_t>(f) * n_chunks * kBins1 + 2 * pair;
            for (int c = 0; c < n_chunks; ++c) { a += p[static_cast<size_t>(c) * kBins1]; b += p[static_cast<size_t>(c) * kBins1 + 1]; }
        } else if (slot < live)
            for (int c = 0; c < n_chunks; ++c) {
                const uint32_t *p = partial + (static_cast<size_t>(f) * n_chunks + c) * pstride + (pass == 1 ? 0 : slot * kSlotStride) + 2 * pair;
                a += p[0]; b += p[1];
            }
        gbuf[i] = static_cast<int64_t>(static_cast<uint64_t>(a) | (static_cast<uint64_t>(b) << 32));
    }
}
constexpr size_t align16(size_t v) { return (v + 15) & ~static_cast<size_t>(15); }

}

size_t radix_state_bytes(int F, int B) {
    const size_t f = static_cast<size_t>(F);
    return align16(f * kBins1 * 2) + align16(f * 2 * 258 * 2) + align16(f * 2 * 512 * 8) + align16(f * 4 * 4) + align16(f * B * 2) +
           2 * align16(f * B * 4) + align16(f * kChunksN * 4);
}
size_t radix_list_bytes(int n, int F) { return sizeof(uint32_t) * (static_cast<size_t>(F) * (static_cast<size_t>(n) / 4 + 64) + 64); }
size_t radix_partial_bytes(int F) {
    const size_t a = static_cast<size_t>(F) * kChunks1 * kBins1, b = static_cast<size_t>(F) * kChunksN * kMaxTargets * kSlotStride;
    return sizeof(uint32_t) * (a > b ? a : b);
}
int radix_max_targets() { return kMaxTargets; }
size_t radix_exchange_words(int F) { return static_cast<size_t>(kMaxTargets) * F * (kSlotStride / 2); }
size_t radix_global_partial_bytes(int F) { return sizeof(uint32_t) * static_cast<size_t>(F) * kMaxTargets * kSlotStride; }

int radix_select(const uint32_t *kt, int n, int F, const int64_t *cum, int B, void *state, uint32_t *partial, uint32_t *lists,
                 uint32_t *thr_keys, hipStream_t s, const RadixComm *comm, int pass1_chunks, uint32_t *le_out) {
    char *p = static_cast<char *>(state);
    auto take = [&](size_t bytes) { char *q = p; p += align16(bytes); return q; };
    const size_t f = static_cast<size_t>(F);
    RadixState st;
    st.map1 = reinterpret_cast<uint16_t *>(take(f * kBins1 * 2));
    st.child_off = reinterpret_cast<uint16_t *>(take(f * 2 * 258 * 2));
    st.child_bits = reinterpret_cast<uint64_t *>(take(f * 2 * 512 * 8));
    st.n_slots = reinterpret_cast<uint32_t *>(take(f * 4 * 4));
    st.tgt_slot = reinterpret_cast<uint16_t *>(take(f * B * 2));
    st.tgt_rank = reinterpret_cast<uint32_t *>(take(f * B * 4));
    st.tgt_prefix = reinterpret_cast<uint32_t *>(take(f * B * 4));
    st.list_cnt = reinterpret_cast<uint32_t *>(take(f * kChunksN * 4));
    st.lists = lists;
    const size_t aux = kBins1 * 2 + 2 * 512 * 8 + 2 * 260 * 2 + kFiltWords * 4 + (kRadixThreads / 64) * 128 * 4;
    const size_t lds1 = static_cast<size_t>(kCopies1) * kBins1 * 4 + aux, lds23 = static_cast<size_t>(kMaxTargets) * 128 * 4 + aux,
                 lds4 = static_cast<size_t>(kMaxTargets) * 64 * 4 + aux;
    static PerDeviceOnce attr;
    if (attr.first()) {
        (void)hipFuncSetAttribute(reinterpret_cast<const void *>(k_radix_count<2>), hipFuncAttributeMaxDynamicSharedMemorySize, static_cast<int>(lds23));
        (void)hipFuncSetAttribute(reinterpret_cast<const void *>(k_radix_count<3>), hipFuncAttributeMaxDynamicSharedMemorySize, static_cast<int>(lds23));
        (void)hipFuncSetAttribute(reinterpret_cast<const void *>(k_radix_count<4>), hipFuncAttributeMaxDynamicSharedMemorySize, static_cast<int>(lds4));
        (void)hipFuncSetAttribute(reinterpret_cast<const void *>(k_radix_targets), hipFuncAttributeMaxDynamicSharedMemorySize, kMaxTargets * 128 * 4);
    }
    int cn = 1;
    if (n >= (1 << 16)) { cn = 2; while (cn < kChunksN && cn * F < 256) cn *= 2; }
    const int c1 = n >= (1 << 16) ? kChunks1 : 1;
    st.list_cap = static_cast<uint32_t>((n / 4) / cn);
    std::vector<uint32_t> h_slots;
    auto finish_pass = [&](int pass, int n_chunks_pass) -> int {
        const uint32_t *src = partial;
        int chunks = n_chunks_pass;
        int p1_u16 = (pass == 1 && pass1_chunks > 0) ? 1 : 0;
        if (comm) {
            int rows = 1;
            hipLaunchKernelGGL(k_radix_globalize, dim3(1024), dim3(256), 0, s, pass, partial, n_chunks_pass, F, st, comm->gbuf, p1_u16);
            p1_u16 = 0;
            if (comm->stream_ordered) {
                if (pass >= 2) rows = std::min(B, kMaxTargets);
            } else {
                if (pass >= 2) {
                    h_slots.resize(static_cast<size_t>(F) * 4);
                    if (hipMemcpyAsync(h_slots.data(), st.n_slots, sizeof(uint32_t) * h_slots.size(), hipMemcpyDeviceToHost, s) != hipSuccess) return 1;
                }
                if (hipStreamSynchronize(s) != hipSuccess) return 1;
                if (pass >= 2) {
                    rows = 0;
                    for (int f2 = 0; f2 < F; ++f2) rows = std::max(rows, static_cast<int>(h_slots[f2 * 4 + (pass - 2)]));
                }
            }
            const size_t words = static_cast<size_t>(rows) * F * (radix_bins(pass) / 2);
            if (comm->allreduce_sum_i64(comm->ctx, comm->gbuf, words) != 0) return 2;
            chunks = 1;
        }
        const size_t lds = pass == 1 ? kBins1 * 4 : static_cast<size_t>(kMaxTargets) * radix_bins(pass) * 4;
        hipLaunchKernelGGL(k_radix_targets, dim3(F), dim3(kTgtThreads), lds, s, pass, src, chunks, cum, B, st, thr_keys, p1_u16, le_out,
                           comm ? comm->gbuf : nullptr, F);
        return 0;
    };
    int rc = 0;
    const bool plain_loads = [] { const char *e = hooks::raw(hooks::RADIX_PLAIN_LOADS); return e && e[0] == '1'; }();
    if (pass1_chunks > 0) {
        if ((rc = finish_pass(1, pass1_chunks)) != 0) return rc;
    } else {
        hipLaunchKernelGGL(k_radix_count<1>, dim3(c1, F), dim3(kRadixThreads), lds1, s, kt, n, c1, B, st, partial, plain_loads);
        if ((rc = finish_pass(1, c1)) != 0) return rc;
    }
    hipLaunchKernelGGL(k_radix_count<2>, dim3(cn, F), dim3(kRadixThreads), lds23, s, kt, n, cn, B, st, partial, plain_loads);
    if ((rc = finish_pass(2, cn)) != 0) return rc;
    hipLaunchKernelGGL(k_radix_count<3>, dim3(cn, F), dim3(kRadixThreads), lds23, s, kt, n, cn, B, st, partial, plain_loads);
    if ((rc = finish_pass(3, cn)) != 0) return rc;
    hipLaunchKernelGGL(k_radix_count<4>, dim3(cn, F), dim3(kRadixThreads), lds4, s, kt, n, cn, B, st, partial, plain_loads);
    return finish_pass(4, cn);
}

int transpose_keys_count(const float *obs, int n, int F, uint32_t *kt, uint32_t *partial, hipStream_t s) {
    const char *env_off = hooks::raw(hooks::TRANSPOSE_COUNT);
    const bool off = env_off && env_off[0] == '0';
    const int chunks = (n + kTcChunk - 1) / kTcChunk;
    if (off || n < (1 << 16) || (n & 3) || (F & 3) || chunks > kTcMaxChunks || (reinterpret_cast<uintptr_t>(obs) & 15) ||
        (reinterpret_cast<uintptr_t>(kt) & 15))
        return 0;
    const size_t lds = sizeof(uint32_t) * (16 * (kBins1 / 2) + kTcWaves * 16 * kTcPatch);
    static PerDeviceOnce attr;
    static uint64_t unsupported = 0;
    int dev = 0;
    (void)hipGetDevice(&dev);
    const uint64_t bit = (dev >= 0 && dev < 64) ? (1ull << dev) : 0;
    if (attr.first() && hipFuncSetAttribute(reinterpret_cast<const void *>(k_transpose_count), hipFuncAttributeMaxDynamicSharedMemorySize, static_cast<int>(lds)) != hipSuccess) {
        (void)hipGetLastError();
        unsupported |= bit;
    }
    if (unsupported & bit) return 0;
    hipLaunchKernelGGL(k_transpose_count, dim3(chunks, (F + 15) / 16), dim3(kTcThreads), lds, s, obs, n, F, kt,
                       reinterpret_cast<uint16_t *>(partial), chunks);
    if (hipGetLastError() != hipSuccess) { unsupported |= bit; return 0; }
    return chunks;
}

}
}
```

Baseline: 541.1.

## Fuse oblivious argmax with split resolution and emit float thresholds from radix select

For oblivious trees without collectives, the separate argmax and resolve_splits kernels are merged into one kernel. Partial blocks compute their argmax and a last-block ticket performs the resolve and publish, removing one launch and one dependency per level. Separately, the final radix-select pass now writes float thresholds directly, which skips a later key-to-float conversion step. The fused path depends on atomic ticketing, agent-scope loads and a reset ticket counter, which adds complexity and a single-block tail.

New measurement: 525.2. 0.971x the previous value.

```diff
diff --git a/gbrl_amd/csrc/engine_candidates.hip b/gbrl_amd/csrc/engine_candidates.hip
--- a/gbrl_amd/csrc/engine_candidates.hip
+++ b/gbrl_amd/csrc/engine_candidates.hip
@@ -588,7 +588,9 @@
                     comm.partial_global = static_cast<uint32_t *>(d_radix_global_.ensure(kern::radix_global_partial_bytes(F)));
                 }
                 uint32_t *d_le = has_coll_ ? nullptr : static_cast<uint32_t *>(d_root_le_.ensure(sizeof(uint32_t) * (static_cast<size_t>(F) * B + F)));
-                const int rc = kern::radix_select(d_kt, N, F, d_cum, B, d_rs, d_rp, d_rl, d_thrkeys, s, has_coll_ ? &comm : nullptr, pass1_chunks, d_le);
+                float *d_thr_fused = (has_coll_ || hooks::on(hooks::UNFUSED_LEVEL_TAIL) ) ? nullptr : d_thr;
+                const int rc = kern::radix_select(d_kt, N, F, d_cum, B, d_rs, d_rp, d_rl, d_thrkeys, s, has_coll_ ? &comm : nullptr, pass1_chunks, d_le, d_thr_fused);
+                floats_done = d_thr_fused != nullptr;
                 root_le_ = d_le;
                 if (rc != 0) throw HipError(rc == 2 ? "allreduce failed" : "radix select failed");
                 last_quantile_fallback_ = false;
diff --git a/gbrl_amd/csrc/engine_grow_levels.hip b/gbrl_amd/csrc/engine_grow_levels.hip
--- a/gbrl_amd/csrc/engine_grow_levels.hip
+++ b/gbrl_amd/csrc/engine_grow_levels.hip
@@ -349,15 +349,22 @@
         kern::score_candidates(L.d_hist, L.d_hist_prev, depth > 0 ? L.d_sub_par : nullptr, L.d_sub_sib, n_act, Fp, NB, D, t.slots, L.lvl_slots, c.d_thr, B, n_cand, model.meta.min_data_in_leaf, c.cosine ? 1 : 0,
                                c.d_scales, L.d_path_len, L.d_path_slot, L.d_path_val, L.d_path_bin, w.scores, w.parent, t.cand_w, t.cand_ref, L.d_isroot,
                                oblivious ? nullptr : w.am_v, w.am_i, s, L.lvl_lo, !L.drop_derived, oblivious ? nullptr : w.am_s, oblivious ? nullptr : w.am_n);
-    if (oblivious)
+    const bool fused_select = oblivious && !has_coll_ && kern::argmax_resolve_supported(n_act) && !hooks::on(hooks::UNFUSED_LEVEL_TAIL) ;
+    if (oblivious && !fused_select)
         kern::argmax(w.scores, n_act, n_cand, t.cand_w, t.cand_ref, w.parent, L.d_isroot, oblivious, w.am_v, w.am_i, res.best_idx(), res.best_score(), s, w.am_s);
     const bool publish_in_resolve = !has_coll_ && !event_results;
     const uint32_t seq = event_results ? 0 : next_seq();
     const bool near_level = w.am_s != nullptr && publish_in_resolve;
     const kern::NearDetect near_detect{w.am_s, oblivious ? nullptr : w.am_n, dims.near_rel, w.parent, L.d_isroot, c.cosine ? 1 : 0, N};
-    kern::resolve_splits(w.am_v, w.am_i, oblivious ? dims.am_parts : L.lvl_slots, res.best_idx(), res.best_score(), oblivious, n_act, t.ref_to_internal, t.cand_slot, t.slots, L.d_hist, nullptr, Fp, NB, D, w.resolved,
-                         res.counts(), max_front, L.d_seg_starts, w.cursors, c.d_thrkeys, B, s, publish_in_resolve ? w.h_res_dev : nullptr, w.d_flag, seq, w.d_pub_done,
-                         L.drop_derived ? L.d_hist_prev : nullptr, L.drop_derived ? L.d_sub_par : nullptr, L.drop_derived ? L.d_sub_sib : nullptr, near_level ? &near_detect : nullptr);
+    if (fused_select)
+        kern::argmax_resolve(w.scores, n_act, n_cand, t.cand_w, t.cand_ref, w.am_v, w.am_i, w.am_s, w.d_pub_done + 1 , res.best_idx(), res.best_score(),
+                             t.ref_to_internal, t.cand_slot, t.slots, L.d_hist, Fp, NB, D, w.resolved, res.counts(), max_front, L.d_seg_starts, w.cursors, c.d_thrkeys, B, s,
+                             publish_in_resolve ? w.h_res_dev : nullptr, w.d_flag, seq, L.drop_derived ? L.d_hist_prev : nullptr, L.drop_derived ? L.d_sub_par : nullptr,
+                             L.drop_derived ? L.d_sub_sib : nullptr, near_level ? &near_detect : nullptr);
+    else
+        kern::resolve_splits(w.am_v, w.am_i, oblivious ? dims.am_parts : L.lvl_slots, res.best_idx(), res.best_score(), oblivious, n_act, t.ref_to_internal, t.cand_slot, t.slots, L.d_hist, nullptr, Fp, NB, D, w.resolved,
+                             res.counts(), max_front, L.d_seg_starts, w.cursors, c.d_thrkeys, B, s, publish_in_resolve ? w.h_res_dev : nullptr, w.d_flag, seq, w.d_pub_done,
+                             L.drop_derived ? L.d_hist_prev : nullptr, L.drop_derived ? L.d_sub_par : nullptr, L.drop_derived ? L.d_sub_sib : nullptr, near_level ? &near_detect : nullptr);
     if (has_coll_) {
         if (!L.ar_level) {
             const int n_win = oblivious ? 1 : n_act;
diff --git a/gbrl_amd/csrc/hooks.h b/gbrl_amd/csrc/hooks.h
--- a/gbrl_amd/csrc/hooks.h
+++ b/gbrl_amd/csrc/hooks.h
@@ -58,7 +58,8 @@
     X(TEST_CAT_CLASH) \
     X(TEST_SMALL_GROW_FAIL) \
     X(TRANSPOSE_COUNT) \
-    X(TRANSPOSE_PLAIN)
+    X(TRANSPOSE_PLAIN) \
+    X(UNFUSED_LEVEL_TAIL)
 
 enum Id : int {
 #define X(n) n,
diff --git a/gbrl_amd/csrc/kernels.h b/gbrl_amd/csrc/kernels.h
--- a/gbrl_amd/csrc/kernels.h
+++ b/gbrl_amd/csrc/kernels.h
@@ -139,7 +139,8 @@
 int radix_select(const uint32_t *kt, int n, int F, const int64_t *cum, int B, void *state, uint32_t *partial, uint32_t *lists,
                  uint32_t *thr_keys, hipStream_t s, const RadixComm *comm ,
                  int pass1_chunks = 0 ,
-                 uint32_t *le_out = nullptr );
+                 uint32_t *le_out = nullptr ,
+                 float *thr_floats = nullptr );
 int transpose_keys_count(const float *obs, int n, int F, uint32_t *kt, uint32_t *partial, hipStream_t s);
 void bin_cols(const uint32_t *kt, int n, int F, const uint32_t *thr_keys, int B, uint16_t *codes, hipStream_t s);
 void scatter_cat_codes_grouped(const uint16_t *cat_codes, int n, int Fc, int F, uint16_t *codes, hipStream_t s);
@@ -201,6 +202,12 @@
                     unsigned *pub_done = nullptr ,
                     const int64_t *hist_prev = nullptr, const int32_t *sub_par = nullptr ,
                     const int32_t *sub_sib = nullptr, const NearDetect *near = nullptr);
+bool argmax_resolve_supported(int n_nodes);
+void argmax_resolve(const float *scores, int n_nodes, int n_cand, const float *cand_weight, const int32_t *cand_ref, float *part_v, int32_t *part_i,
+                    float *part_s , unsigned *ticket, int32_t *best_idx, float *best_score, const int32_t *ref_to_internal, const int32_t *cand_slot,
+                    const FeatureSlot *slots, const int64_t *hist_local, int Fp, int NB, int D, NodeSplit *out, int64_t *counts4 , int max_front,
+                    const int32_t *seg_start, int32_t *cursors, const uint32_t *thr_keys, int B, hipStream_t s, void *pub, uint32_t *pub_flag, uint32_t pub_seq,
+                    const int64_t *hist_prev, const int32_t *sub_par, const int32_t *sub_sib, const NearDetect *near);
 
 constexpr int kNearCands = 16;
 constexpr int kNearMaxRows = 65536;
diff --git a/gbrl_amd/csrc/kernels.hip b/gbrl_amd/csrc/kernels.hip
--- a/gbrl_amd/csrc/kernels.hip
+++ b/gbrl_amd/csrc/kernels.hip
@@ -986,15 +986,14 @@
 }
 
 constexpr int kArgmaxThreads = 256;
-__global__ __launch_bounds__(kArgmaxThreads) void k_argmax_stage1(const float *__restrict__ scores, int n_nodes, int n_cand,
-                                                                  const float *__restrict__ w, const int32_t *__restrict__ ref,
-                                                                  const float *__restrict__ parent, const int32_t *__restrict__ is_root,
-                                                                  int oblivious, float *__restrict__ part_v, int32_t *__restrict__ part_i,
-                                                                  float *__restrict__ part_s ) {
-    const int j = blockIdx.x * kArgmaxThreads + threadIdx.x;
-    const int node = blockIdx.y;
+__device__ __forceinline__ void argmax_part(const float *__restrict__ scores, int n_nodes, int n_cand, const float *__restrict__ w,
+                                            const int32_t *__restrict__ ref, const float *__restrict__ parent, const int32_t *__restrict__ is_root,
+                                            int oblivious, int node, int part, int n_parts, int t , int base,
+                                            float *sv, float *s2, int *si, float *__restrict__ part_v, int32_t *__restrict__ part_i,
+                                            float *__restrict__ part_s ) {
+    const int j = part * kArgmaxThreads + t;
     Best mine{-INFINITY, 0x7fffffff};
-    if (j < n_cand) {
+    if (part < n_parts && j < n_cand) {
         float sc;
         if (oblivious) {
             sc = 0.0f;
@@ -1014,53 +1013,64 @@
         }
         mine = better(mine, Best{sc, ref[j]});
     }
+    sv[base + t] = mine.v;
+    si[base + t] = mine.i;
+    s2[base + t] = -INFINITY;
+    __syncthreads();
+    for (int o = kArgmaxThreads / 2; o > 0; o >>= 1) {
+        if (t < o) {
+            Best a2{sv[base + t], si[base + t]}, b2{sv[base + t + o], si[base + t + o]};
+            s2[base + t] = second_distinct(a2.v, s2[base + t], b2.v, s2[base + t + o]);
+            a2 = better(a2, b2);
+            sv[base + t] = a2.v;
+            si[base + t] = a2.i;
+        }
+        __syncthreads();
+    }
+    if (t == 0 && part < n_parts) {
+        part_v[static_cast<size_t>(node) * n_parts + part] = sv[base];
+        part_i[static_cast<size_t>(node) * n_parts + part] = si[base];
+        if (part_s) part_s[static_cast<size_t>(node) * n_parts + part] = s2[base];
+    }
+}
+__global__ __launch_bounds__(kArgmaxThreads) void k_argmax_stage1(const float *__restrict__ scores, int n_nodes, int n_cand,
+                                                                  const float *__restrict__ w, const int32_t *__restrict__ ref,
+                                                                  const float *__restrict__ parent, const int32_t *__restrict__ is_root,
+                                                                  int oblivious, float *__restrict__ part_v, int32_t *__restrict__ part_i,
+                                                                  float *__restrict__ part_s ) {
     __shared__ float sv[kArgmaxThreads], s2[kArgmaxThreads];
     __shared__ int si[kArgmaxThreads];
-    sv[threadIdx.x] = mine.v;
-    si[threadIdx.x] = mine.i;
-    s2[threadIdx.x] = -INFINITY;
-    __syncthreads();
-    for (int o = kArgmaxThreads / 2; o > 0; o >>= 1) {
-        if (threadIdx.x < o) {
-            Best a2{sv[threadIdx.x], si[threadIdx.x]}, b2{sv[threadIdx.x + o], si[threadIdx.x + o]};
-            s2[threadIdx.x] = second_distinct(a2.v, s2[threadIdx.x], b2.v, s2[threadIdx.x + o]);
-            a2 = better(a2, b2);
-            sv[threadIdx.x] = a2.v;
-            si[threadIdx.x] = a2.i;
-        }
-        __syncthreads();
-    }
-    if (threadIdx.x == 0) {
-        part_v[static_cast<size_t>(node) * gridDim.x + blockIdx.x] = sv[0];
-        part_i[static_cast<size_t>(node) * gridDim.x + blockIdx.x] = si[0];
-        if (part_s) part_s[static_cast<size_t>(node) * gridDim.x + blockIdx.x] = s2[0];
-    }
-}
-__global__ __launch_bounds__(64) void k_resolve_splits(const float *__restrict__ part_v, const int32_t *__restrict__ part_i, int n_parts,
-                                                       int32_t *__restrict__ best_idx, float *__restrict__ best_score, int oblivious,
-                                                       const int32_t *__restrict__ ref_to_internal, const int32_t *__restrict__ cand_slot,
-                                                       const FeatureSlot *__restrict__ slots, const int64_t *__restrict__ hist_local,
-                                                       const int64_t *__restrict__ hist_global, int Fp, int NB, int D,
-                                                       NodeSplit *__restrict__ out, int64_t *__restrict__ counts4, int max_front,
-                                                       const int32_t *__restrict__ seg_start , int32_t *__restrict__ cursors,
-                                                       const uint32_t *__restrict__ thr_keys, int B, char *pub, uint32_t *pub_flag,
-                                                       uint32_t pub_seq, unsigned *pub_done, const int64_t *__restrict__ hist_prev,
-                                                       const int32_t *__restrict__ sub_par, const int32_t *__restrict__ sub_sib,
-                                                       const float *__restrict__ part_s, const int32_t *__restrict__ part_n , float near_rel, const float *__restrict__ parent,
-                                                       const int32_t *__restrict__ is_root, int cosine_score, long long near_rows) {
-    const int node = blockIdx.x;
-    int32_t *pub_idx = reinterpret_cast<int32_t *>(pub);
-    float *pub_score = reinterpret_cast<float *>(pub + 4 * static_cast<size_t>(max_front));
-    int64_t *pub_counts = reinterpret_cast<int64_t *>(pub + 8 * static_cast<size_t>(max_front));
-    const int src_node = oblivious ? 0 : node;
+    argmax_part(scores, n_nodes, n_cand, w, ref, parent, is_root, oblivious, blockIdx.y, blockIdx.x, gridDim.x, threadIdx.x, 0, sv, s2, si, part_v, part_i, part_s);
+}
+
+struct ResolveArgs {
+    const float *part_v; const int32_t *part_i; int n_parts;
+    int32_t *best_idx; float *best_score; int oblivious;
+    const int32_t *ref_to_internal; const int32_t *cand_slot; const FeatureSlot *slots;
+    const int64_t *hist_local; const int64_t *hist_global; int Fp, NB, D;
+    NodeSplit *out; int64_t *counts4; int max_front;
+    const int32_t *seg_start ; int32_t *cursors; const uint32_t *thr_keys; int B;
+    char *pub; uint32_t *pub_flag; uint32_t pub_seq; unsigned *pub_done;
+    const int64_t *hist_prev; const int32_t *sub_par; const int32_t *sub_sib;
+    const float *part_s; const int32_t *part_n ; float near_rel; const float *parent; const int32_t *is_root;
+    int cosine_score; long long near_rows;
+};
+struct Winner { Best best; float second; };
+template <bool FRESH>
+__device__ __forceinline__ Winner resolve_winner(const ResolveArgs &a, int src_node, int lane) {
+    const float *part_v = a.part_v, *part_s = a.part_s;
+    const int32_t *part_i = a.part_i, *part_n = a.part_n;
+    const int n_parts = a.n_parts;
+    auto ldf = [](const float *p) { return FRESH ? __hip_atomic_load(p, __ATOMIC_RELAXED, __HIP_MEMORY_SCOPE_AGENT) : *p; };
+    auto ldi = [](const int32_t *p) { return FRESH ? __hip_atomic_load(p, __ATOMIC_RELAXED, __HIP_MEMORY_SCOPE_AGENT) : *p; };
     Best mine{-INFINITY, 0x7fffffff};
     float second = -INFINITY;
     int mine_nr = 0;
-    for (int q = threadIdx.x; q < n_parts; q += kWave) {
-        const Best other{part_v[static_cast<size_t>(src_node) * n_parts + q], part_i[static_cast<size_t>(src_node) * n_parts + q]};
+    for (int q = lane; q < n_parts; q += kWave) {
+        const Best other{ldf(part_v + static_cast<size_t>(src_node) * n_parts + q), ldi(part_i + static_cast<size_t>(src_node) * n_parts + q)};
         if (part_s) {
-            const int onr = part_n ? part_n[static_cast<size_t>(src_node) * n_parts + q] : 0;
-            second = second_merge(mine.v, mine_nr, second, other.v, onr, part_s[static_cast<size_t>(src_node) * n_parts + q]);
+            const int onr = part_n ? ldi(part_n + static_cast<size_t>(src_node) * n_parts + q) : 0;
+            second = second_merge(mine.v, mine_nr, second, other.v, onr, ldf(part_s + static_cast<size_t>(src_node) * n_parts + q));
             if (better_takes_second(mine, other)) mine_nr = onr;
         }
         mine = better(mine, other);
@@ -1074,19 +1084,32 @@
         }
         mine = better(mine, other);
     }
-    const int best = mine.i == 0x7fffffff ? 0 : mine.i;
-    const float best_v = mine.v;
-    if (threadIdx.x == 0 && node == src_node && !hist_global) {
+    return Winner{mine, second};
+}
+__device__ __forceinline__ void resolve_node(const ResolveArgs &a, int node, int src_node, int lane, const Winner &win) {
+    const int oblivious = a.oblivious, Fp = a.Fp, NB = a.NB, D = a.D, max_front = a.max_front, B = a.B;
+    const int64_t *hist_local = a.hist_local, *hist_global = a.hist_global, *hist_prev = a.hist_prev;
+    const int32_t *sub_par = a.sub_par, *sub_sib = a.sub_sib, *is_root = a.is_root;
+    const float *part_s = a.part_s, *parent = a.parent;
+    int64_t *counts4 = a.counts4;
+    char *pub = a.pub;
+    int32_t *pub_idx = reinterpret_cast<int32_t *>(pub);
+    float *pub_score = reinterpret_cast<float *>(pub + 4 * static_cast<size_t>(max_front));
+    int64_t *pub_counts = reinterpret_cast<int64_t *>(pub + 8 * static_cast<size_t>(max_front));
+    const float second = win.second;
+    const int best = win.best.i == 0x7fffffff ? 0 : win.best.i;
+    const float best_v = win.best.v;
+    if (lane == 0 && node == src_node && !hist_global) {
         counts4[3 * static_cast<size_t>(max_front) + node] = __float_as_int(second);
         if (pub) pub_counts[3 * static_cast<size_t>(max_front) + node] = __float_as_int(second);
     }
-    if (threadIdx.x == 0 && node == src_node) {
-        best_idx[node] = best; best_score[node] = best_v;
+    if (lane == 0 && node == src_node) {
+        a.best_idx[node] = best; a.best_score[node] = best_v;
         if (pub) { pub_idx[node] = best; pub_score[node] = best_v; }
     }
-    const int j = ref_to_internal[best];
-    const int fs = cand_slot[j];
-    const FeatureSlot sl = slots[fs];
+    const int j = a.ref_to_internal[best];
+    const int fs = a.cand_slot[j];
+    const FeatureSlot sl = a.slots[fs];
     const int bin = sl.is_cat ? (j - sl.cand_base + 1) : (j - sl.cand_base);
     const int W = D + 1;
     const int NBe = min(NB, sl.n_cand + 1);
@@ -1101,7 +1124,7 @@
             sub = sib >= 0 ? hist_local + (static_cast<size_t>(sib) * Fp + fs) * NB * W : nullptr;
         }
         long long tot = 0, right = 0;
-        for (int c0 = threadIdx.x; c0 < NBe; c0 += 8 * kWave) {
+        for (int c0 = lane; c0 < NBe; c0 += 8 * kWave) {
             long long n[8];
 #pragma unroll
             for (int u = 0; u < 8; ++u) { const int c = c0 + u * kWave; n[u] = c < NBe ? src[c * W + D] : 0; }
@@ -1117,7 +1140,7 @@
             }
         }
         for (int o = kWave / 2; o > 0; o >>= 1) { tot += __shfl_xor(tot, o, kWave); right += __shfl_xor(right, o, kWave); }
-        if (threadIdx.x == 0) {
+        if (lane == 0) {
             counts4[(2 * pass + 0) * static_cast<size_t>(max_front) + node] = tot;
             counts4[(2 * pass + 1) * static_cast<size_t>(max_front) + node] = right;
             if (pub) {
@@ -1131,35 +1154,69 @@
                     float mag;
                     if (oblivious) mag = fabsf(best_v);
                     else { const float par = is_root[node] ? 0.0f : parent[node]; mag = fmaxf(fabsf(best_v + par), fabsf(par)); }
-                    const float win = near_window_rel(near_rel, oblivious ? near_rows : tot) * mag;
+                    const float win = near_window_rel(a.near_rel, oblivious ? a.near_rows : tot) * mag;
                     if (second != -INFINITY && best_v - second <= win) near = 1;
-                    if (!oblivious && !is_root[node] && fabsf(best_v) <= win && !(cosine_score == 0 && (right == 0 || right == tot))) near = 1;
+                    if (!oblivious && !is_root[node] && fabsf(best_v) <= win && !(a.cosine_score == 0 && (right == 0 || right == tot))) near = 1;
                 }
                 counts4[2 * static_cast<size_t>(max_front) + node] = near;
                 if (pub) pub_counts[2 * static_cast<size_t>(max_front) + node] = near;
             }
         }
     }
-    if (threadIdx.x == 0) {
+    if (lane == 0) {
         NodeSplit q{};
         q.fslot = fs; q.bin = bin; q.is_cat = sl.is_cat;
-        q.thr_key = (!sl.is_cat && thr_keys) ? thr_keys[static_cast<size_t>(fs) * B + bin] : 0u;
-        if (seg_start) {
+        q.thr_key = (!sl.is_cat && a.thr_keys) ? a.thr_keys[static_cast<size_t>(fs) * B + bin] : 0u;
+        if (a.seg_start) {
             const float bs = best_v;
             q.do_split = oblivious ? (bs != -INFINITY) : (bs >= 0.0f);
-            q.seg_start = seg_start[node];
+            q.seg_start = a.seg_start[node];
             q.n_left = n_left;
-            cursors[2 * node] = 0;
-            cursors[2 * node + 1] = 0;
-        }
-        out[node] = q;
-        if (pub) {
-            __threadfence_system();
-            if (atomicAdd(pub_done, 1u) == gridDim.x - 1) {
-                *pub_done = 0;
-                __hip_atomic_store(pub_flag, pub_seq, __ATOMIC_RELEASE, __HIP_MEMORY_SCOPE_SYSTEM);
-            }
-        }
+            a.cursors[2 * node] = 0;
+            a.cursors[2 * node + 1] = 0;
+        }
+        a.out[node] = q;
+    }
+}
+__global__ __launch_bounds__(64) void k_resolve_splits(const ResolveArgs a) {
+    const int node = blockIdx.x, src_node = a.oblivious ? 0 : node;
+    const Winner win = resolve_winner<false>(a, src_node, threadIdx.x);
+    resolve_node(a, node, src_node, threadIdx.x, win);
+    if (threadIdx.x == 0 && a.pub) {
+        __threadfence_system();
+        if (atomicAdd(a.pub_done, 1u) == gridDim.x - 1) {
+            *a.pub_done = 0;
+            __hip_atomic_store(a.pub_flag, a.pub_seq, __ATOMIC_RELEASE, __HIP_MEMORY_SCOPE_SYSTEM);
+        }
+    }
+}
+
+constexpr int kResolveParts = 4, kResolveThreads = kResolveParts * kArgmaxThreads, kResolveNodes = 2 * (kResolveThreads / kWave);
+__global__ __launch_bounds__(kResolveThreads) void k_argmax_resolve(const float *__restrict__ scores, int n_nodes, int n_cand, const float *__restrict__ w,
+                                                                    const int32_t *__restrict__ ref, float *part_v, int32_t *part_i, float *part_s ,
+                                                                    unsigned *ticket , const ResolveArgs a) {
+    __shared__ float sv[kResolveThreads], s2[kResolveThreads];
+    __shared__ int si[kResolveThreads];
+    __shared__ int s_last;
+    const int t = threadIdx.x & (kArgmaxThreads - 1), base = threadIdx.x - t;
+    argmax_part(scores, n_nodes, n_cand, w, ref, nullptr, nullptr, 1, 0, blockIdx.x * kResolveParts + base / kArgmaxThreads, a.n_parts, t, base, sv, s2, si,
+                part_v, part_i, part_s);
+    if (t == 0) __threadfence();
+    __syncthreads();
+    if (threadIdx.x == 0) s_last = atomicAdd(ticket, 1u) == gridDim.x - 1;
+    __syncthreads();
+    if (!s_last) return;
+    __threadfence();
+    const int lane = threadIdx.x & (kWave - 1), wave = threadIdx.x / kWave;
+    if (wave < n_nodes) {
+        const Winner win = resolve_winner<true>(a, 0, lane);
+        for (int node = wave; node < n_nodes; node += kResolveThreads / kWave) resolve_node(a, node, 0, lane, win);
+        if (lane == 0 && a.pub) __threadfence_system();
+    }
+    __syncthreads();
+    if (threadIdx.x == 0) {
+        *ticket = 0;
+        if (a.pub) __hip_atomic_store(a.pub_flag, a.pub_seq, __ATOMIC_RELEASE, __HIP_MEMORY_SCOPE_SYSTEM);
     }
 }
 
@@ -1663,15 +1720,42 @@
                        is_root, oblivious ? 1 : 0, part_v, part_i, part_s);
     (void)best_idx; (void)best_score;
 }
+static ResolveArgs resolve_args(const float *part_v, const int32_t *part_i, int n_parts, int32_t *best_idx, float *best_score, bool oblivious, const int32_t *ref_to_internal,
+                                const int32_t *cand_slot, const FeatureSlot *slots, const int64_t *hist_local, const int64_t *hist_global, int Fp, int NB, int D,
+                                NodeSplit *out, int64_t *counts4, int max_front, const int32_t *seg_start, int32_t *cursors, const uint32_t *thr_keys,
+                                int B, void *pub, uint32_t *pub_flag, uint32_t pub_seq, unsigned *pub_done, const int64_t *hist_prev,
+                                const int32_t *sub_par, const int32_t *sub_sib, const NearDetect *near) {
+    ResolveArgs a{};
+    a.part_v = part_v; a.part_i = part_i; a.n_parts = n_parts; a.best_idx = best_idx; a.best_score = best_score; a.oblivious = oblivious ? 1 : 0;
+    a.ref_to_internal = ref_to_internal; a.cand_slot = cand_slot; a.slots = slots; a.hist_local = hist_local; a.hist_global = hist_global;
+    a.Fp = Fp; a.NB = NB; a.D = D; a.out = out; a.counts4 = counts4; a.max_front = max_front; a.seg_start = seg_start; a.cursors = cursors;
+    a.thr_keys = thr_keys; a.B = B; a.pub = static_cast<char *>(pub); a.pub_flag = pub_flag; a.pub_seq = pub_seq; a.pub_done = pub_done;
+    a.hist_prev = hist_prev; a.sub_par = sub_par; a.sub_sib = sub_sib;
+    a.part_s = near ? near->part_s : nullptr; a.part_n = near ? near->part_n : nullptr; a.near_rel = near ? near->rel : 0.0f;
+    a.parent = near ? near->parent : nullptr; a.is_root = near ? near->is_root : nullptr; a.cosine_score = near ? near->cosine : 1; a.near_rows = near ? near->rows : 0;
+    return a;
+}
 void resolve_splits(const float *part_v, const int32_t *part_i, int n_parts, int32_t *best_idx, float *best_score, bool oblivious, int n_nodes, const int32_t *ref_to_internal, const int32_t *cand_slot,
                     const FeatureSlot *slots, const int64_t *hist_local, const int64_t *hist_global, int Fp, int NB, int D,
                     NodeSplit *out, int64_t *counts4, int max_front, const int32_t *seg_start, int32_t *cursors, const uint32_t *thr_keys,
                     int B, hipStream_t s, void *pub, uint32_t *pub_flag, uint32_t pub_seq, unsigned *pub_done, const int64_t *hist_prev,
                     const int32_t *sub_par, const int32_t *sub_sib, const NearDetect *near) {
-    hipLaunchKernelGGL(k_resolve_splits, dim3(n_nodes), dim3(64), 0, s, part_v, part_i, n_parts, best_idx, best_score, oblivious ? 1 : 0,
-                       ref_to_internal, cand_slot, slots, hist_local, hist_global, Fp, NB, D, out, counts4, max_front, seg_start, cursors, thr_keys, B,
-                       static_cast<char *>(pub), pub_flag, pub_seq, pub_done, hist_prev, sub_par, sub_sib,
-                       near ? near->part_s : nullptr, near ? near->part_n : nullptr, near ? near->rel : 0.0f, near ? near->parent : nullptr, near ? near->is_root : nullptr, near ? near->cosine : 1, near ? near->rows : 0);
+    const ResolveArgs a = resolve_args(part_v, part_i, n_parts, best_idx, best_score, oblivious, ref_to_internal, cand_slot, slots, hist_local, hist_global, Fp, NB, D, out, counts4,
+                                       max_front, seg_start, cursors, thr_keys, B, pub, pub_flag, pub_seq, pub_done, hist_prev, sub_par, sub_sib, near);
+    hipLaunchKernelGGL(k_resolve_splits, dim3(n_nodes), dim3(64), 0, s, a);
+}
+bool argmax_resolve_supported(int n_nodes) { return n_nodes <= kResolveNodes; }
+void argmax_resolve(const float *scores, int n_nodes, int n_cand, const float *w, const int32_t *ref, float *part_v, int32_t *part_i, float *part_s, unsigned *ticket,
+                    int32_t *best_idx, float *best_score, const int32_t *ref_to_internal, const int32_t *cand_slot,
+                    const FeatureSlot *slots, const int64_t *hist_local, int Fp, int NB, int D,
+                    NodeSplit *out, int64_t *counts4, int max_front, const int32_t *seg_start, int32_t *cursors, const uint32_t *thr_keys,
+                    int B, hipStream_t s, void *pub, uint32_t *pub_flag, uint32_t pub_seq, const int64_t *hist_prev,
+                    const int32_t *sub_par, const int32_t *sub_sib, const NearDetect *near) {
+    const int parts = argmax_parts(n_cand);
+    const ResolveArgs a = resolve_args(part_v, part_i, parts, best_idx, best_score, true, ref_to_internal, cand_slot, slots, hist_local, nullptr, Fp, NB, D, out, counts4,
+                                       max_front, seg_start, cursors, thr_keys, B, pub, pub_flag, pub_seq, nullptr, hist_prev, sub_par, sub_sib, near);
+    hipLaunchKernelGGL(k_argmax_resolve, dim3((parts + kResolveParts - 1) / kResolveParts), dim3(kResolveThreads), 0, s, scores, n_nodes, n_cand, w, ref, part_v, part_i,
+                       part_s, ticket, a);
 }
 
 __global__ void k_localize_splits(NodeSplit *__restrict__ splits, const int32_t *__restrict__ n_local,
diff --git a/gbrl_amd/csrc/radix_select.hip b/gbrl_amd/csrc/radix_select.hip
--- a/gbrl_amd/csrc/radix_select.hip
+++ b/gbrl_amd/csrc/radix_select.hip
@@ -1,4 +1,5 @@
 #include "kernels.h"
+#include "kernels_common.h"
 #include "hooks.h"
 
 #include <algorithm>
@@ -281,7 +282,8 @@
 __global__ __launch_bounds__(kTgtThreads) void k_radix_targets(int pass, const uint32_t *__restrict__ partial, int n_chunks,
                                                                const int64_t *__restrict__ cum, int B, RadixState st,
                                                                uint32_t *__restrict__ thr_keys, int p1_u16, uint32_t *__restrict__ le_out,
-                                                               const int64_t *__restrict__ gbuf , int F) {
+                                                               const int64_t *__restrict__ gbuf , int F,
+                                                               float *__restrict__ thr_out ) {
     extern __shared__ uint32_t sums[];
     __shared__ int tslot[kMaxTargets], tdig[kMaxTargets];
     __shared__ uint32_t scratch[16], total_slots;
@@ -355,7 +357,11 @@
         if (pass == 4 && le_out) le_out[static_cast<size_t>(f) * B + k] = prefix < 0x007fffffu ? le_out[static_cast<size_t>(gridDim.x) * B + f] : le_here;
     }
     if (pass == 4) {
-        if (k < B) thr_keys[static_cast<size_t>(f) * B + k] = prefix;
+        if (k < B) {
+            if (thr_out && prefix < 0x007fffffu) prefix = 0x007fffffu;
+            thr_keys[static_cast<size_t>(f) * B + k] = prefix;
+            if (thr_out) thr_out[static_cast<size_t>(f) * B + k] = key_to_float(prefix);
+        }
         return;
     }
     if (k < kMaxTargets) { tslot[k] = k < B ? slot : -1; tdig[k] = digit; }
@@ -429,7 +435,7 @@
 size_t radix_global_partial_bytes(int F) { return sizeof(uint32_t) * static_cast<size_t>(F) * kMaxTargets * kSlotStride; }
 
 int radix_select(const uint32_t *kt, int n, int F, const int64_t *cum, int B, void *state, uint32_t *partial, uint32_t *lists,
-                 uint32_t *thr_keys, hipStream_t s, const RadixComm *comm, int pass1_chunks, uint32_t *le_out) {
+                 uint32_t *thr_keys, hipStream_t s, const RadixComm *comm, int pass1_chunks, uint32_t *le_out, float *thr_floats) {
     char *p = static_cast<char *>(state);
     auto take = [&](size_t bytes) { char *q = p; p += align16(bytes); return q; };
     const size_t f = static_cast<size_t>(F);
@@ -485,7 +491,7 @@
         }
         const size_t lds = pass == 1 ? kBins1 * 4 : static_cast<size_t>(kMaxTargets) * radix_bins(pass) * 4;
         hipLaunchKernelGGL(k_radix_targets, dim3(F), dim3(kTgtThreads), lds, s, pass, src, chunks, cum, B, st, thr_keys, p1_u16, le_out,
-                           comm ? comm->gbuf : nullptr, F);
+                           comm ? comm->gbuf : nullptr, F, pass == 4 ? thr_floats : nullptr);
         return 0;
     };
     int rc = 0;
```
